# imjaegyun/Traffic-Context-Augmented-Vehicle-Trajectory-Prediction-Framework-Using-Multimodal-LLM

Hardware: AMD Instinct MI355X
Metric: trajectories/sec (higher is better)
Workload: dtype f16

## Files before the change

### include/tcavt.h

```cpp
#ifndef TCAVT_H
#define TCAVT_H

#include <stdint.h>

#ifdef __cplusplus
extern "C" {
#endif

typedef void* tcavt_stream_t;

#define TCAVT_ABI_VERSION 5

#define TCAVT_OK 0
#define TCAVT_ERR_ARG 1
#define TCAVT_ERR_HIP 2
#define TCAVT_ERR_ARCH 3

#define TCAVT_F32 0
#define TCAVT_BF16 1
#define TCAVT_F16 2

int tcavt_abi_version(void);
const char* tcavt_last_error(void);
int tcavt_init(int device, int* num_cus);
// ... 58 lines not shown

int tcavt_gemm_bf16(const tcavt_gemm_args* args, tcavt_stream_t stream);

int tcavt_rmsnorm(const float* x, const float* gamma, float eps, void* out_bf16,
                  float* out_f32, int M, int H, void* out_drop_bf16, float dropout_p,
                  uint64_t dropout_seed, uint32_t dropout_site, int dtype16 ,
                  tcavt_stream_t stream);

int tcavt_layernorm(const float* x, const float* residual, const float* gamma,
                    const float* beta, float eps, float* out_f32, void* out_bf16,
                    int M, int D, int dtype16 , tcavt_stream_t stream);

int tcavt_dropout(const void* x, void* out, int64_t n, int dtype, float p, uint64_t seed, uint32_t site,
                  const void* add ,
                  tcavt_stream_t stream);

int tcavt_set_dropout_epoch(const uint64_t* epoch_dev);
int tcavt_dropout_epoch_advance(uint64_t* epoch_dev, tcavt_stream_t stream);

int tcavt_copy_batch(void* const* dst, const void* const* src, const int64_t* bytes, int n, tcavt_stream_t stream);

int tcavt_cast_f32_16(const float* x, void* out16, int64_t n, int dtype16, tcavt_stream_t stream);

int tcavt_embed_fuse(const void* table_bf16, const int64_t* ids, const float* img,
                     const float* vis_mod, const float* txt_mod, float* h, int B,
                     int Nq, int Lt, int H, int V, int* bad_id_flag, int table_dtype,
                     void* h16, float* part, int npart, float stream_scale ,
                     tcavt_stream_t stream);

int tcavt_mask_to_kvlen(const int64_t* mask, int B, int Lt, int Nq, int32_t* kv_len,
                        int* not_prefix_flag, tcavt_stream_t stream);

int tcavt_attn_causal_gqa(const void* qkv, void* out, const int32_t* kv_len, int B,
                          int L, int nq, int nkv, float scale, int dtype16, tcavt_stream_t stream);
int tcavt_attn_causal_gqa_lse(const void* qkv, void* out, float* lse, const int32_t* kv_len, int B,
                              int L, int nq, int nkv, float scale, int dtype16, tcavt_stream_t stream);

int tcavt_softmax_rows(const float* S, int64_t lds, void* P, int64_t ldp, int out_dtype, int rows,
                       int n_valid, int n_out, float dropout_p, uint64_t dropout_seed, uint32_t dropout_site,
                       tcavt_stream_t stream);

int tcavt_mha(const void* q, int64_t ldq, const void* k, int64_t ldk, const void* v,
              int64_t ldv, void* out, int64_t ldo, const int32_t* key_len, int B,
              int Lq, int Lk, int nh, int dh, float scale, int in_dtype,
              int out_dtype, float dropout_p, uint64_t dropout_seed, uint32_t dropout_site,
              tcavt_stream_t stream);

int tcavt_gemm_f32(const float* A, int64_t lda, const float* W, int64_t ldw,
                   const float* bias, const float* residual, int64_t ldr, float* C,
                   int64_t ldc, int M, int N, int K, int flags, float dropout_p,
                   uint64_t dropout_seed, uint32_t dropout_site, tcavt_stream_t stream);

int tcavt_poly_embed(const float* polygon, const float* w_in, const float* b_in,
                     const float* pos, float* x, int B, int P, int D,
                     tcavt_stream_t stream);
int tcavt_masked_mean(const float* enc, const int32_t* len, float* emb, int B, int P,
                      int D, tcavt_stream_t stream);

int tcavt_ltsf_front(const float* x, const float* conv_w, const float* conv_b,
                     const float* enc_w, const float* enc_b, const float* pos,
                     float* enc_tok, float* xp_tok ,
                     int B, int C, int T, tcavt_stream_t stream);

int tcavt_ltsf_decode(const float* e_tok, const float* dec_w, const float* dec_b,
                      const float* lane_adj, float* dec, int B, int C, int T, int To,
                      tcavt_stream_t stream);

int tcavt_transpose_ct(const float* in, float* out_f32, void* out_bf16, int B, int C,
                       int To, int dtype16, tcavt_stream_t stream);

int tcavt_out_head(const float* fused, const float* w, const float* bias,
                   const float* x, float* out, int B, int To, int C, int F, int T,
                   int add_last, tcavt_stream_t stream);

int tcavt_traj_metrics(const float* pred, const float* gt, const float* norm_stat,
                       float* sums, int32_t* argmin, float* per_sample, int B, int K,
                       int To, tcavt_stream_t stream);

int tcavt_gemm_f32_strided(const float* A, int64_t rsA, int64_t csA, const float* W, int64_t rsW,
                           int64_t csW, const float* bias, const float* residual, int64_t ldr, float* C,
                           int64_t ldc, int M, int N, int K, int flags, float* ws, int64_t ws_elems,
                           tcavt_stream_t stream);


int tcavt_transpose16(const void* in, int64_t ld_in, void* out, int64_t ld_out, int rows, int cols,
                      int rows_pad, int batch, int64_t s_in, int64_t s_out, int f16_to_bf16, tcavt_stream_t stream);
int tcavt_transpose_f32_bf16(const float* in, int64_t ld_in, void* out, int64_t ld_out, int rows,
                             int cols, int rows_pad, tcavt_stream_t stream);
int tcavt_colsum(const void* g, int64_t ld, int dtype, float* out, int M, int N, int accumulate,
                 float* ws, int64_t ws_elems, tcavt_stream_t stream);
int tcavt_relu_bwd(float* g, const void* y, int y_dtype, int64_t n, tcavt_stream_t stream);
int tcavt_add_inplace(float* a, const float* b, int64_t n, tcavt_stream_t stream);
int tcavt_silu_mul_bwd(const void* gu_bf16, const void* g_act_bf16, void* g_gu_bf16, int64_t M, int I, int dtype16,
                       tcavt_stream_t stream);
int tcavt_rmsnorm_bwd(const void* x, const float* gamma, const void* gy_bf16, const void* gy2_bf16, float eps,
                      float* gx, void* gx_bf16, int accumulate, int M, int H, int gy_dtype, int out_dtype,
                      const float* gy_scale, int x_dtype, tcavt_stream_t stream);
int tcavt_grad_scale_pick(const void* g_a, const void* g_b, int64_t n, int dtype16, float target, float* scale,
                          uint32_t* scratch, const int32_t* backoff, tcavt_stream_t stream);
int tcavt_rope_bwd_pack(const float* g32, void* out_bf16, const float* rope_cos, const float* rope_sin, int64_t M,
                        int ncols, int rope_cols, int L, int dtype16, tcavt_stream_t stream);
int tcavt_attn_causal_gqa_bwd(const void* qkv_bf16, const void* dO_bf16, float* g32, const int32_t* kv_len, int B, int T,
                              int nq, int nkv, int head_dim, float scale, tcavt_stream_t stream);
int tcavt_causal_softmax_bwd_rows(const float* S, const float* dP, void* P_bf16, void* dS_bf16, const int32_t* kv_len,
                                  int B, int T, int Tp, int nq, float scale, tcavt_stream_t stream);
int tcavt_causal_softmax_bwd_tiles(const float* S, const float* dP, void* dS_bf16, void* PT_bf16, void* dST_bf16,
                                   const int32_t* kv_len, int B, int T, int Tp, int nq, float scale, tcavt_stream_t stream);
int tcavt_attn_bwd_scores(const void* qkv_bf16, const void* dO_bf16, void* dS_bf16, void* PT_bf16, void* dST_bf16,
                          float* dQ, int64_t ld_dq, float* stats, const int32_t* kv_len, int B, int T, int Tp, int nq,
                          int nkv, int head_dim, float scale, int dtype16, const float* lse, const void* att,
                          tcavt_stream_t stream);
int tcavt_attn_bwd_resident_ok(int T, int nq, int nkv);
int tcavt_attn_bwd_resident(const void* qkv16, const void* dO16, const void* att16, const float* lse, void* g_qkv16,
                            float* stats, const float* rope_cos, const float* rope_sin, const int32_t* kv_len, int B, int T,
                            int nq, int nkv, int head_dim, float scale, int dtype16, tcavt_stream_t stream);
int tcavt_attn_bwd_long_ok(int T, int nq, int nkv);
int tcavt_attn_bwd_long(const void* qkv16, const void* dO16, const void* att16, const float* lse, void* g_qkv16, float* stats,
                        const float* rope_cos, const float* rope_sin, const int32_t* kv_len, int B, int T, int nq, int nkv,
                        int head_dim, float scale, int dtype16, tcavt_stream_t stream);
int tcavt_attn_bwd_dkv(const void* qkv_bf16, const void* dO_bf16, const float* stats, float* g32, const int32_t* kv_len,
                       int B, int T, int Tp, int nq, int nkv, int head_dim, float scale, int dtype16, tcavt_stream_t stream);
int tcavt_gqa_rope_bwd_pack(const float* G3, void* out_bf16, const float* rope_cos, const float* rope_sin, int64_t M,
                            int nq, int nkv, int head_dim, int L, tcavt_stream_t stream);
int tcavt_wgrad_tn(const void* G, int64_t ldg, int g_col0, int n, const void* X, int64_t ldx, int x_dtype, float* C,
                   int64_t ldc, int M, int H, int trans_out, int g_dtype, const float* rs_part, int rs_npart, int rs_h,
                   float rs_eps, tcavt_stream_t stream);
int tcavt_lora_wgrad_a(const void* x16, const float* part, int npart, float eps, const float* gamma, const void* g_t, float* dA,
                       int64_t ldc, int M, int H, float dropout_p, uint64_t dropout_seed, uint32_t site_q, uint32_t site_v,
                       int dtype16, tcavt_stream_t stream);

int tcavt_clip_grad_norm(float* g, int64_t n, float max_norm, float grad_scale, float* scratch, tcavt_stream_t stream);
int tcavt_layernorm_bwd(const float* x, const float* gamma, const float* gy, float eps, float* gx,
                        float* ggamma, float* gbeta, int M, int D, float* ws, int64_t ws_elems, tcavt_stream_t stream);
int tcavt_mha_bwd(const float* q, int64_t ldq, const float* k, int64_t ldk, const float* v, int64_t ldv,
                  const float* go, int64_t ldo, float* gq, float* gk, float* gv, int64_t ldg,
                  const int32_t* key_len, int B, int Lq, int Lk, int nh, int dh, float scale,
                  float dropout_p, uint64_t dropout_seed, uint32_t dropout_site,
                  tcavt_stream_t stream);
int tcavt_softmax_bwd_rows(const void* P_f16, int64_t ldp, const float* dP, int64_t ldd, void* dS_bf16,
                           int64_t lds, float scale, int rows, int n_valid, int n_out,
                           tcavt_stream_t stream);
int tcavt_mse_grad(const float* pred, const float* gt, const float* norm_stat, float* g, int B, int To,
                   tcavt_stream_t stream);
int tcavt_mse_grad_seeded(const float* pred, const float* gt, const float* norm_stat, const float* g_loss,
                          const float* g_pred, float* g, int B, int To, tcavt_stream_t stream);
int tcavt_out_head_bwd(const float* g, const float* fused, const float* w, float* gf, float* gw, float* gb,
                       int B, int To, int C, int F, tcavt_stream_t stream);
int tcavt_nlinear_bwd(const float* in_tok, const float* W, const float* g, int64_t g_sb, int64_t g_sc,
                      int64_t g_ss, float* gW, float* gbias, float* gin_tok, int B, int C, int T, int S,
                      tcavt_stream_t stream);
int tcavt_conv1x1_bwd(const float* gxp_tok, const float* x, float* gw, float* gb, int B, int C, int T,
                      int F, tcavt_stream_t stream);
int tcavt_poly_embed_bwd(const float* g, const float* polygon, float* gw, float* gb, float* gpos, int B,
                         int P, int D, tcavt_stream_t stream);
int tcavt_masked_mean_bwd(const float* gemb, const int32_t* len, float* genc, int B, int P, int D,
                          tcavt_stream_t stream);
int tcavt_adamw(float* p, const float* g, float* m, float* v, int64_t n, float lr, float beta1, float beta2,
                float eps, float weight_decay, int step, float grad_scale, tcavt_stream_t stream);

typedef struct tcavt_llama_layer {
  const void* w_qkv;
  const void* a_cat;
  const void* b_ext;
  const void* w_o;
  const void* w_gu;
  const void* w_d;
  float* tape_h_mid;
  float* tape_h_out;
  void* tape_qkv;
  void* tape_gu;
  void* tape_t;
  void* tape_att;
  float* tape_lse;
  float* tape_part;
} tcavt_llama_layer;

typedef struct tcavt_llama_stack_args {
  const tcavt_llama_layer* layers;
  const float* gamma_final;
  const float* rope_cos;
  const float* rope_sin;
  float* h;
  void* h16;
  float* part;
  const int32_t* kv_len;
  void* qkv;
  void* att;
  void* act;
  void* t;
  void* xq;
  void* xv;
  float* out_f32;
  void* out16;
  void* k_cache;
  void* v_cache;
  void* const* events;
  int32_t n_layers, B, L, H, I, nq, nkv, dtype16;
  int32_t kv_lmax;
  int32_t gemm_tile;
  int32_t npart_in;
  float stream_scale;
  float rms_eps, lora_scale;
  float lora_dropout_p;
  uint32_t lora_first_site;
  uint64_t dropout_seed;
  int32_t* nonfinite_flag;
  void* splitk_ws;
  int64_t splitk_ws_bytes;
} tcavt_llama_stack_args;
// ... 377 lines not shown
```

### traffic-context-augmented-vehicle-trajectory-prediction-framework-using-multimodal-llm_amd/capi.py

```python
import ctypes
import os

import torch

_HERE = os.path.dirname(os.path.abspath(__file__))
LIB_PATH = os.path.join(_HERE, "libtcavt_hip.so")

ABI_VERSION = 5
F32, BF16, F16 = 0, 1, 2
EPI_BIAS, EPI_RELU, EPI_RESIDUAL, EPI_SILU_MUL, EPI_ROPE, EPI_BIAS_ROW, EPI_ACCUM = 1, 2, 4, 8, 16, 32, 64
EPI_NORM_OUT, EPI_ROWSCALE, EPI_SILU_BWD = 128, 256, 512
ACT_A_FRAG16, ACT_OUT_FRAG16, ACT_BLOCK8 = 1, 2, 4
W_FRAG16 = 1

c_void_p, c_int, c_int64, c_float = ctypes.c_void_p, ctypes.c_int, ctypes.c_int64, ctypes.c_float


class GemmArgs(ctypes.Structure):

    _fields_ = [
        ("A", c_void_p), ("lda", c_int64),
        ("W", c_void_p), ("ldw", c_int64),
        ("A2", c_void_p), ("lda2", c_int64),
        ("W2", c_void_p), ("ldw2", c_int64),
        ("C", c_void_p), ("ldc", c_int64),
        ("bias", c_void_p),
        ("residual", c_void_p), ("ldr", c_int64),
        ("rope_cos", c_void_p),
        ("rope_sin", c_void_p),
        ("M", ctypes.c_int32), ("N", ctypes.c_int32), ("K", ctypes.c_int32), ("K2", ctypes.c_int32),
        ("out_dtype", ctypes.c_int32),
        ("epilogue", ctypes.c_int32),
        ("rope_L", ctypes.c_int32), ("rope_cols", ctypes.c_int32),
        ("tile", ctypes.c_int32),
        ("acc_scale", ctypes.c_float),
        ("in_dtype", ctypes.c_int32),
        ("batch", ctypes.c_int32), ("batch_inner", ctypes.c_int32),
        ("sAo", c_int64), ("sAi", c_int64), ("sWo", c_int64), ("sWi", c_int64), ("sCo", c_int64), ("sCi", c_int64),
        ("dropout_p", ctypes.c_float), ("dropout_site", ctypes.c_uint32), ("dropout_seed", ctypes.c_uint64),
        ("batch_w_group", ctypes.c_int32), ("w_layout", ctypes.c_int32),
        ("silu_preact", c_void_p), ("ld_preact", c_int64),
        ("norm_h16", c_void_p), ("norm_part", c_void_p), ("rowscale_part", c_void_p),
        ("rowscale_npart", ctypes.c_int32), ("rowscale_h", ctypes.c_int32), ("rowscale_eps", ctypes.c_float),
        ("norm_scale", ctypes.c_float),
        ("rope_pos", c_void_p),
        ("nonfinite_flag", c_void_p), ("nonfinite_tag", ctypes.c_int32), ("act_layout", ctypes.c_int32),
        ("norm_res16", c_void_p), ("splitk_ws", c_void_p), ("splitk_ws_bytes", c_int64),
        ("lora_part", c_void_p), ("lora_part_a", c_void_p), ("lora_part_lda", c_int64), ("lora_part_np", c_int),
        ("lora_part_scale", c_float),
    ]


class LlamaLayer(ctypes.Structure):

    _fields_ = [(n, c_void_p) for n in ("w_qkv", "a_cat", "b_ext", "w_o", "w_gu", "w_d", "tape_h_mid", "tape_h_out",
                                        "tape_qkv", "tape_gu", "tape_t", "tape_att", "tape_lse", "tape_part")]


TLAYER_FIELDS = ("w_in", "b_in", "w_out", "b_out", "w_q", "b_q", "w_kv", "b_kv", "w_co", "b_co", "w1", "b1", "w2", "b2",
                 "n1_w", "n1_b", "n2_w", "n2_b", "n3_w", "n3_b",
                 "qkv", "att", "y", "x1", "x1b", "cq", "ckv", "catt", "cy", "x2", "x2b", "ffh", "y2", "out", "outb")


class TLayer(ctypes.Structure):

    _fields_ = [(n, c_void_p) for n in TLAYER_FIELDS]


class TStackArgs(ctypes.Structure):

    _fields_ = [
        ("layers", ctypes.POINTER(TLayer)),
        ("x", c_void_p), ("xb", c_void_p), ("mem", c_void_p), ("memb", c_void_p), ("key_len", c_void_p),
        ("n_layers", ctypes.c_int32), ("B", ctypes.c_int32), ("L", ctypes.c_int32), ("Lk", ctypes.c_int32),
        ("E", ctypes.c_int32), ("FF", ctypes.c_int32), ("nhead", ctypes.c_int32), ("dtype16", ctypes.c_int32),
        ("dropout_p", ctypes.c_float), ("first_site", ctypes.c_uint32), ("dropout_seed", ctypes.c_uint64),
    ]


class CrossAttnArgs(ctypes.Structure):

    _fields_ = [(n, c_void_p) for n in ("q", "wk_t", "w_v", "b_v", "fh", "fh_t", "qp", "scores", "probs", "ctx", "att")] + [
        (n, ctypes.c_int32) for n in ("B", "To", "L", "Lp", "H", "nhead", "dtype16")] + [
        ("dropout_p", ctypes.c_float), ("dropout_site", ctypes.c_uint32), ("reserved0", ctypes.c_uint32),
        ("dropout_seed", ctypes.c_uint64)]


class TLayerGrads(ctypes.Structure):

    _fields_ = [(n, c_void_p) for n in ("g_w_in", "g_b_in", "g_w_out", "g_b_out", "g_w1", "g_b1", "g_w2", "g_b2", "g_n1_w", "g_n1_b",
                                        "g_n2_w", "g_n2_b")]


class TStackBwdArgs(ctypes.Structure):

    _fields_ = [("fwd", ctypes.POINTER(TStackArgs)), ("grads", ctypes.POINTER(TLayerGrads))] + [(n, c_void_p) for n in (
        "g_out", "g_x", "g_tmp", "g_y2", "g_y2d", "g_x1", "g_y", "g_yd", "g_att", "g_f", "g_qkv")] + [
        ("red_ws", c_void_p), ("red_ws_elems", c_int64)]
# ... 62 lines not shown
        ("g_h", c_void_p), ("g_hb", c_void_p), ("g_xn", c_void_p), ("g_xl", c_void_p), ("g_att", c_void_p),
        ("g_qkv0", c_void_p), ("g_qkv1", c_void_p), ("g_t0", c_void_p), ("g_t1", c_void_p),
        ("dA", c_void_p), ("dB", c_void_p), ("stats", c_void_p),
        ("leaf_stream", c_void_p), ("events", ctypes.POINTER(c_void_p)),
        ("n_layers", ctypes.c_int32), ("B", ctypes.c_int32), ("L", ctypes.c_int32), ("H", ctypes.c_int32),
        ("I", ctypes.c_int32), ("nq", ctypes.c_int32), ("nkv", ctypes.c_int32), ("dtype16", ctypes.c_int32),
        ("npart", ctypes.c_int32), ("lora_rank", ctypes.c_int32), ("input_grad", ctypes.c_int32), ("reserved0", ctypes.c_int32),
        ("rms_eps", ctypes.c_float), ("lora_scale", ctypes.c_float), ("lora_dropout_p", ctypes.c_float),
        ("lora_first_site", ctypes.c_uint32), ("dropout_seed", ctypes.c_uint64), ("scale_backoff", c_void_p),
    ]


class SampleParams(ctypes.Structure):

    _fields_ = [("temperature", c_float), ("top_p", c_float), ("repetition_penalty", c_float), ("top_k", ctypes.c_int32),
                ("no_repeat_ngram_size", ctypes.c_int32), ("do_sample", ctypes.c_int32), ("eos_token_id", c_int64),
                ("pad_token_id", c_int64), ("seed", ctypes.c_uint64)]


class DecodeArgs(ctypes.Structure):

    _fields_ = [("layers", ctypes.POINTER(LlamaLayer))] + [(n, c_void_p) for n in (
        "gamma_final", "rope_cos", "rope_sin", "table", "txt_mod", "cur_tok", "pos", "h", "h16", "part", "qkv", "att", "act",
        "t", "k_cache", "v_cache", "x16", "logits", "bad_id_flag")] + [(n, ctypes.c_int32) for n in (
            "n_layers", "B", "H", "I", "nq", "nkv", "V", "dtype16", "kv_lmax", "rope_L")] + [
        ("rms_eps", c_float), ("lora_scale", c_float), ("nonfinite_flag", c_void_p), ("splitk_ws", c_void_p),
        ("splitk_ws_bytes", c_int64), ("lora_part", c_void_p), ("lora_rank", c_int), ("stream_scale", ctypes.c_float),
        ("w_layout", ctypes.c_int32), ("act_layout", ctypes.c_int32), ("table_packed", c_void_p)]


class LmLossArgs(ctypes.Structure):

    _fields_ = [("h16", c_void_p), ("ldh", c_int64), ("table", c_void_p), ("table_t", c_void_p), ("ldt", c_int64),
                ("labels", c_void_p), ("kv_len", c_void_p)] + [(n, ctypes.c_int32) for n in (
                    "B", "L", "V", "H", "Nq", "dtype16", "grad_dtype", "reserved0")] + [(n, c_void_p) for n in (
                        "loss", "count", "lse", "row_loss", "flag", "g_loss", "g_out")] + [
        ("ldg", c_int64), ("workspace", c_void_p), ("workspace_bytes", c_int64)]


class LmEvalArgs(ctypes.Structure):

    _fields_ = [("h16", c_void_p), ("ldh", c_int64), ("table", c_void_p), ("labels", c_void_p), ("kv_len", c_void_p)] + [
        (n, ctypes.c_int32) for n in ("B", "L", "V", "H", "Nq", "dtype16")] + [(n, c_void_p) for n in (
            "loss", "count", "lse", "row_loss", "flag", "pred", "correct", "sample_tokens", "sample_correct", "sample_nll")] + [
        ("workspace", c_void_p), ("workspace_bytes", c_int64)]


_SIGNATURES = {
    "tcavt_abi_version": [],
    "tcavt_last_error": [],
    "tcavt_init": [c_int, ctypes.POINTER(c_int)],
    "tcavt_gemm_bf16": [ctypes.POINTER(GemmArgs), c_void_p],
    "tcavt_rmsnorm": [c_void_p, c_void_p, c_float, c_void_p, c_void_p, c_int, c_int, c_void_p, c_float, ctypes.c_uint64,
                      ctypes.c_uint32, c_int, c_void_p],
    "tcavt_layernorm": [c_void_p, c_void_p, c_void_p, c_void_p, c_float, c_void_p, c_void_p, c_int, c_int, c_int, c_void_p],
    "tcavt_cast_f32_16": [c_void_p, c_void_p, c_int64, c_int, c_void_p],
    "tcavt_copy_batch": [c_void_p, c_void_p, c_void_p, c_int, c_void_p],
    "tcavt_embed_fuse": [c_void_p, c_void_p, c_void_p, c_void_p, c_void_p, c_void_p, c_int, c_int, c_int, c_int,
                         c_int, c_void_p, c_int, c_void_p, c_void_p, c_int, c_float, c_void_p],
    "tcavt_softmax_rows": [c_void_p, c_int64, c_void_p, c_int64, c_int, c_int, c_int, c_int, c_float, ctypes.c_uint64,
                           ctypes.c_uint32, c_void_p],
    "tcavt_set_dropout_epoch": [c_void_p],
    "tcavt_dropout_epoch_advance": [c_void_p, c_void_p],
    "tcavt_dropout": [c_void_p, c_void_p, c_int64, c_int, c_float, ctypes.c_uint64, ctypes.c_uint32, c_void_p, c_void_p],
    "tcavt_mask_to_kvlen": [c_void_p, c_int, c_int, c_int, c_void_p, c_void_p, c_void_p],
    "tcavt_attn_causal_gqa": [c_void_p, c_void_p, c_void_p, c_int, c_int, c_int, c_int, c_float, c_int, c_void_p],
    "tcavt_attn_causal_gqa_lse": [c_void_p, c_void_p, c_void_p, c_void_p, c_int, c_int, c_int, c_int, c_float, c_int, c_void_p],
    "tcavt_mha": [c_void_p, c_int64, c_void_p, c_int64, c_void_p, c_int64, c_void_p, c_int64, c_void_p, c_int,
                  c_int, c_int, c_int, c_int, c_float, c_int, c_int, c_float, ctypes.c_uint64, ctypes.c_uint32, c_void_p],
    "tcavt_gemm_f32": [c_void_p, c_int64, c_void_p, c_int64, c_void_p, c_void_p, c_int64, c_void_p, c_int64,
                       c_int, c_int, c_int, c_int, c_float, ctypes.c_uint64, ctypes.c_uint32, c_void_p],
    "tcavt_poly_embed": [c_void_p, c_void_p, c_void_p, c_void_p, c_void_p, c_int, c_int, c_int, c_void_p],
    "tcavt_masked_mean": [c_void_p, c_void_p, c_void_p, c_int, c_int, c_int, c_void_p],
    "tcavt_ltsf_front": [c_void_p, c_void_p, c_void_p, c_void_p, c_void_p, c_void_p, c_void_p, c_void_p, c_int, c_int,
                         c_int, c_void_p],
    "tcavt_ltsf_decode": [c_void_p, c_void_p, c_void_p, c_void_p, c_void_p, c_int, c_int, c_int, c_int, c_void_p],
    "tcavt_transpose_ct": [c_void_p, c_void_p, c_void_p, c_int, c_int, c_int, c_int, c_void_p],
    "tcavt_out_head": [c_void_p, c_void_p, c_void_p, c_void_p, c_void_p, c_int, c_int, c_int, c_int, c_int,
                       c_int, c_void_p],
    "tcavt_traj_metrics": [c_void_p, c_void_p, c_void_p, c_void_p, c_void_p, c_void_p, c_int, c_int, c_int,
                           c_void_p],
    "tcavt_gemm_f32_strided": [c_void_p, c_int64, c_int64, c_void_p, c_int64, c_int64, c_void_p, c_void_p, c_int64,
                               c_void_p, c_int64, c_int, c_int, c_int, c_int, c_void_p, c_int64, c_void_p],
    "tcavt_transpose16": [c_void_p, c_int64, c_void_p, c_int64, c_int, c_int, c_int, c_int, c_int64, c_int64, c_int, c_void_p],
    "tcavt_transpose_f32_bf16": [c_void_p, c_int64, c_void_p, c_int64, c_int, c_int, c_int, c_void_p],
    "tcavt_colsum": [c_void_p, c_int64, c_int, c_void_p, c_int, c_int, c_int, c_void_p, c_int64, c_void_p],
    "tcavt_relu_bwd": [c_void_p, c_void_p, c_int, c_int64, c_void_p],
    "tcavt_add_inplace": [c_void_p, c_void_p, c_int64, c_void_p],
    "tcavt_silu_mul_bwd": [c_void_p, c_void_p, c_void_p, c_int64, c_int, c_int, c_void_p],
    "tcavt_rmsnorm_bwd": [c_void_p, c_void_p, c_void_p, c_void_p, c_float, c_void_p, c_void_p, c_int, c_int, c_int, c_int, c_int,
                          c_void_p, c_int, c_void_p],
    "tcavt_lora_dgrad": [c_void_p, c_void_p, c_void_p, c_void_p, c_int, c_int, c_float, ctypes.c_uint64, ctypes.c_uint32,
                         ctypes.c_uint32, c_int, c_void_p],
    "tcavt_grad_scale_pick": [c_void_p, c_void_p, c_int64, c_int, c_float, c_void_p, c_void_p, c_void_p, c_void_p],
    "tcavt_rope_bwd_pack": [c_void_p, c_void_p, c_void_p, c_void_p, c_int64, c_int, c_int, c_int, c_int, c_void_p],
    "tcavt_attn_causal_gqa_bwd": [c_void_p, c_void_p, c_void_p, c_void_p, c_int, c_int, c_int, c_int, c_int, c_float,
                                  c_void_p],
    "tcavt_causal_softmax_bwd_rows": [c_void_p, c_void_p, c_void_p, c_void_p, c_void_p, c_int, c_int, c_int, c_int, c_float,
                                      c_void_p],
    "tcavt_causal_softmax_bwd_tiles": [c_void_p, c_void_p, c_void_p, c_void_p, c_void_p, c_void_p, c_int, c_int, c_int, c_int,
                                       c_float, c_void_p],
    "tcavt_attn_bwd_scores": [c_void_p, c_void_p, c_void_p, c_void_p, c_void_p, c_void_p, c_int64, c_void_p, c_void_p, c_int,
                              c_int, c_int, c_int, c_int, c_int, c_float, c_int, c_void_p, c_void_p, c_void_p],
    "tcavt_attn_bwd_resident_ok": [c_int, c_int, c_int],
    "tcavt_attn_bwd_resident": [c_void_p, c_void_p, c_void_p, c_void_p, c_void_p, c_void_p, c_void_p, c_void_p, c_void_p, c_int,
                                c_int, c_int, c_int, c_int, c_float, c_int, c_void_p],
    "tcavt_attn_bwd_long_ok": [c_int, c_int, c_int],
    "tcavt_attn_bwd_long": [c_void_p, c_void_p, c_void_p, c_void_p, c_void_p, c_void_p, c_void_p, c_void_p, c_void_p, c_int,
                            c_int, c_int, c_int, c_int, c_float, c_int, c_void_p],
    "tcavt_attn_bwd_dkv": [c_void_p, c_void_p, c_void_p, c_void_p, c_void_p, c_int, c_int, c_int, c_int, c_int, c_int, c_float,
                           c_int, c_void_p],
    "tcavt_gqa_rope_bwd_pack": [c_void_p, c_void_p, c_void_p, c_void_p, c_int64, c_int, c_int, c_int, c_int, c_void_p],
    "tcavt_wgrad_tn": [c_void_p, c_int64, c_int, c_int, c_void_p, c_int64, c_int, c_void_p, c_int64, c_int, c_int, c_int, c_int,
                       c_void_p, c_int, c_int, c_float, c_void_p],
    "tcavt_lora_wgrad_a": [c_void_p, c_void_p, c_int, c_float, c_void_p, c_void_p, c_void_p, c_int64, c_int, c_int, c_float,
                           ctypes.c_uint64, ctypes.c_uint32, ctypes.c_uint32, c_int, c_void_p],
    "tcavt_clip_grad_norm": [c_void_p, c_int64, c_float, c_float, c_void_p, c_void_p],
    "tcavt_layernorm_bwd": [c_void_p, c_void_p, c_void_p, c_float, c_void_p, c_void_p, c_void_p, c_int, c_int, c_void_p,
                            c_int64, c_void_p],
    "tcavt_mha_bwd": [c_void_p, c_int64, c_void_p, c_int64, c_void_p, c_int64, c_void_p, c_int64, c_void_p, c_void_p,
                      c_void_p, c_int64, c_void_p, c_int, c_int, c_int, c_int, c_int, c_float, c_float, ctypes.c_uint64,
                      ctypes.c_uint32, c_void_p],
    "tcavt_softmax_bwd_rows": [c_void_p, c_int64, c_void_p, c_int64, c_void_p, c_int64, c_float, c_int, c_int, c_int,
                               c_void_p],
    "tcavt_mse_grad": [c_void_p, c_void_p, c_void_p, c_void_p, c_int, c_int, c_void_p],
    "tcavt_mse_grad_seeded": [c_void_p, c_void_p, c_void_p, c_void_p, c_void_p, c_void_p, c_int, c_int, c_void_p],
    "tcavt_out_head_bwd": [c_void_p, c_void_p, c_void_p, c_void_p, c_void_p, c_void_p, c_int, c_int, c_int, c_int,
                           c_void_p],
    "tcavt_nlinear_bwd": [c_void_p, c_void_p, c_void_p, c_int64, c_int64, c_int64, c_void_p, c_void_p, c_void_p, c_int,
                          c_int, c_int, c_int, c_void_p],
    "tcavt_conv1x1_bwd": [c_void_p, c_void_p, c_void_p, c_void_p, c_int, c_int, c_int, c_int, c_void_p],
    "tcavt_poly_embed_bwd": [c_void_p, c_void_p, c_void_p, c_void_p, c_void_p, c_int, c_int, c_int, c_void_p],
    "tcavt_masked_mean_bwd": [c_void_p, c_void_p, c_void_p, c_int, c_int, c_int, c_void_p],
    "tcavt_adamw": [c_void_p, c_void_p, c_void_p, c_void_p, c_int64, c_float, c_float, c_float, c_float, c_float,
                    c_int, c_float, c_void_p],
    "tcavt_llama_stack_forward": [ctypes.POINTER(LlamaStackArgs), c_void_p],
    "tcavt_sample_logits": [c_void_p, c_int, c_int, c_void_p, c_int, c_void_p, ctypes.POINTER(SampleParams), c_void_p, c_void_p,
                            c_void_p, c_void_p, c_void_p, c_int, c_int, c_void_p, c_int64, c_void_p],
    "tcavt_sample_workspace_bytes": [c_int],
    "tcavt_gather_last": [c_void_p, c_void_p, c_void_p, c_int, c_int, c_int, c_void_p],
    "tcavt_llama_decode_step": [ctypes.POINTER(DecodeArgs), c_void_p],
    "tcavt_norm_npart": [c_int, c_int, c_int],
    "tcavt_pack_weight16": [c_void_p, c_int64, c_void_p, c_int, c_int, c_void_p],
    "tcavt_lora_down": [c_void_p, c_void_p, c_void_p, c_int, c_int, c_float, c_float, ctypes.c_uint64, ctypes.c_uint32,
                        ctypes.c_uint32, c_int, c_void_p],
    "tcavt_rownorm_prep": [c_void_p, c_void_p, c_void_p, c_int64, c_int, c_int, c_int, c_int, c_float, c_void_p],
    "tcavt_allreduce_flat": [c_void_p, c_int64, c_void_p, c_void_p],
    "tcavt_tlayer_stack_forward": [ctypes.POINTER(TStackArgs), c_void_p],
    "tcavt_cross_attn_forward": [ctypes.POINTER(CrossAttnArgs), c_void_p],
    "tcavt_ltsf_forward": [ctypes.POINTER(LtsfArgs), c_int, c_void_p],
    "tcavt_cross_attn_backward": [ctypes.POINTER(CrossAttnBwdArgs), c_void_p],
    "tcavt_ltsf_backward": [ctypes.POINTER(LtsfBwdArgs), c_int, c_void_p],
    "tcavt_tlayer_stack_backward": [ctypes.POINTER(TStackBwdArgs), c_void_p],
    "tcavt_rmsnorm16": [c_void_p, c_void_p, c_float, c_void_p, c_void_p, c_int, c_int, c_int, c_void_p],
    "tcavt_llama_stack_backward": [ctypes.POINTER(LlamaBackwardArgs), c_void_p],
    "tcavt_events_create": [ctypes.POINTER(c_void_p), c_int],
    "tcavt_events_destroy": [ctypes.POINTER(c_void_p), c_int],
    "tcavt_event_elapsed_ms": [c_void_p, c_void_p, ctypes.POINTER(c_float)],
    "tcavt_adamw_gated": [c_void_p, c_void_p, c_void_p, c_void_p, c_int64, c_float, c_float, c_float, c_float, c_float,
                          c_float, c_void_p, c_void_p, c_void_p, c_void_p],
    "tcavt_lm_loss_workspace_bytes": [c_int64, c_int, c_int],
    "tcavt_lm_loss_forward": [ctypes.POINTER(LmLossArgs), c_void_p],
    "tcavt_lm_loss_backward": [ctypes.POINTER(LmLossArgs), c_void_p],
    "tcavt_lm_eval_workspace_bytes": [c_int64, c_int, c_int],
    "tcavt_lm_eval": [ctypes.POINTER(LmEvalArgs), c_void_p],
}
_RESTYPES = {"tcavt_last_error": ctypes.c_char_p, "tcavt_sample_workspace_bytes": c_int64,
             "tcavt_lm_loss_workspace_bytes": c_int64, "tcavt_lm_eval_workspace_bytes": c_int64}

EXPORTED_SYMBOLS = tuple(_SIGNATURES)


class TcavtError(RuntimeError):
    pass


_lib = None


def lib():
    global _lib
    if _lib is not None:
        return _lib
    if not os.path.exists(LIB_PATH):
        raise TcavtError(
            f"{LIB_PATH} not found: the HIP extension is not built. Run "
            "`python -c 'import __graft_entry__ as g; g.build()'` (or `python -m tcavt_amd.build`). "
            "There is no CPU/PyTorch fallback for the hot path."
        )
    handle = ctypes.CDLL(LIB_PATH)
    for name, argtypes in _SIGNATURES.items():
        fn = getattr(handle, name)
        fn.argtypes = argtypes
        fn.restype = _RESTYPES.get(name, c_int)
    if handle.tcavt_abi_version() != ABI_VERSION:
        raise TcavtError("libtcavt_hip.so ABI version mismatch")
    _lib = handle
# ... 28 lines not shown
```

### traffic-context-augmented-vehicle-trajectory-prediction-framework-using-multimodal-llm_amd/csrc/llm_backward.hip

```cpp
#include "common.hpp"
#include "philox.hpp"
#include <stdlib.h>

namespace tcavt {

__device__ __forceinline__ float sigmoid_f(float g) { return __builtin_amdgcn_rcpf(1.f + __expf(-g)); }

template <bool F16>
__device__ __forceinline__ f32x4 mfma16b(const bf16x8& a, const bf16x8& b, const f32x4& c) {
  if constexpr (F16) return __builtin_amdgcn_mfma_f32_16x16x32_f16(__builtin_bit_cast(f16x8, a), __builtin_bit_cast(f16x8, b), c, 0, 0, 0);
  else return __builtin_amdgcn_mfma_f32_16x16x32_bf16(a, b, c, 0, 0, 0);
}
template <bool F16>
__device__ __forceinline__ float half16(unsigned int w, int k) { return k ? from16_hi<F16>(w) : from16_lo<F16>(w); }

template <bool F16>
__global__ __launch_bounds__(256) void silu_mul_bwd_kernel(const bf16_t* __restrict__ gu, const bf16_t* __restrict__ g_act,
                                                           bf16_t* __restrict__ g_gu, long M, int I) {
  const long blk = (long)blockIdx.x * blockDim.x + threadIdx.x;
  const long nblk = M * (I >> 4);
  if (blk >= nblk) return;
  const u32x4* src = reinterpret_cast<const u32x4*>(gu + blk * 32);
  const u32x4* dsrc = reinterpret_cast<const u32x4*>(g_act + blk * 16);
  u32x4 gv[2] = {src[0], src[1]}, uv[2] = {src[2], src[3]}, dv[2] = {dsrc[0], dsrc[1]};
// ... 1424 lines not shown
    for (int b = 0; b < 4; ++b) acc[a][b] = f32x4{0.f, 0.f, 0.f, 0.f};
  const int tp = tid >> 4, cc = (tid & 15) * 16;
  const int grow = tid >> 2, gc0 = (tid & 3) * 8;
  for (int m0 = mbeg; m0 < mend; m0 += 32) {
    {
      u32x4 v[2][2];
#pragma unroll
      for (int r = 0; r < 2; ++r) {
        const int m = m0 + 2 * tp + r;
#pragma unroll
        for (int o = 0; o < 2; ++o) {
          v[r][o] = u32x4{0u, 0u, 0u, 0u};
          if (m < mend && h0 + cc + 8 * o < H) v[r][o] = *reinterpret_cast<const u32x4*>(X + (long)m * H + h0 + cc + 8 * o);
        }
      }
      u32x4 gv = {0u, 0u, 0u, 0u};
      if (tid < 128 && m0 + grow < mend) gv = *reinterpret_cast<const u32x4*>(Gt + (long)(m0 + grow) * 64 + gc0);
      if (tid < 32) rs_s[tid] = m0 + tid < mend ? part_rscale(part + (long)(m0 + tid) * npart, npart, inv_h, eps) : 0.f;
      __syncthreads();
      const float rs2[2] = {rs_s[2 * tp], rs_s[2 * tp + 1]};
#pragma unroll
      for (int o = 0; o < 2; ++o) {
        u32x4 wq[2], wv[2];
#pragma unroll
        for (int r = 0; r < 2; ++r) {
          float sq[8], sv[8];
          if (drop) {
            const unsigned long long oct =
                ((unsigned long long)(m0 + 2 * tp + r) * (unsigned long long)H + (unsigned long long)(h0 + cc + 8 * o)) >> 3;
            dropout_oct(dq, oct, sq);
            dropout_oct(dv, oct, sv);
          }
#pragma unroll
          for (int e = 0; e < 4; ++e) {
            const float lo = from16_lo<F16>(v[r][o][e]) * rs2[r], hi = from16_hi<F16>(v[r][o][e]) * rs2[r];
            wq[r][e] = drop ? pack16x2<F16>(lo * sq[2 * e], hi * sq[2 * e + 1]) : pack16x2<F16>(lo, hi);
            if (drop) wv[r][e] = pack16x2<F16>(lo * sv[2 * e], hi * sv[2 * e + 1]);
          }
        }
#pragma unroll
        for (int e = 0; e < 4; ++e) {
          const int c = cc + 8 * o + 2 * e;
          *reinterpret_cast<unsigned int*>(&xq[c * XS + 2 * tp]) = (wq[0][e] & 0xffffu) | (wq[1][e] << 16);
          *reinterpret_cast<unsigned int*>(&xq[(c + 1) * XS + 2 * tp]) = (wq[0][e] >> 16) | (wq[1][e] & 0xffff0000u);
          if (drop) {
            *reinterpret_cast<unsigned int*>(&xv[c * XS + 2 * tp]) = (wv[0][e] & 0xffffu) | (wv[1][e] << 16);
            *reinterpret_cast<unsigned int*>(&xv[(c + 1) * XS + 2 * tp]) = (wv[0][e] >> 16) | (wv[1][e] & 0xffff0000u);
          }
        }
      }
      if (tid < 128) {
#pragma unroll
        for (int e = 0; e < 4; ++e) {
          gt[(gc0 + 2 * e) * XS + grow] = static_cast<bf16_t>(gv[e] & 0xffffu);
          gt[(gc0 + 2 * e + 1) * XS + grow] = static_cast<bf16_t>(gv[e] >> 16);
        }
      }
    }
    __syncthreads();
    const u32x4 aq = *reinterpret_cast<const u32x4*>(&gt[r16 * XS + kq * 8]);
    const u32x4 av = *reinterpret_cast<const u32x4*>(&gt[(16 + r16) * XS + kq * 8]);
#pragma unroll
    for (int b = 0; b < 4; ++b) {
      const int row = (wave * 64 + b * 16 + r16) * XS + kq * 8;
      const u32x4 bq = *reinterpret_cast<const u32x4*>(&xq[row]);
      const u32x4 bv = *reinterpret_cast<const u32x4*>(&xvp[row]);
      acc[0][b] = mfma16b<F16>(__builtin_bit_cast(bf16x8, aq), __builtin_bit_cast(bf16x8, bq), acc[0][b]);
      acc[1][b] = mfma16b<F16>(__builtin_bit_cast(bf16x8, av), __builtin_bit_cast(bf16x8, bv), acc[1][b]);
    }
    __syncthreads();
  }
#pragma unroll
  for (int a = 0; a < 2; ++a)
#pragma unroll
    for (int b = 0; b < 4; ++b) {
      const int h = h0 + wave * 64 + b * 16 + r16;
      if (h >= H) continue;
      const float gm = gamma[h];
#pragma unroll
      for (int e = 0; e < 4; ++e) atomicAdd(dA + (long)(a * 16 + 4 * kq + e) * ldc + h, acc[a][b][e] * gm);
    }
}

template <bool XF16, bool GF16 = false>
__global__ __launch_bounds__(256) void wgrad_tn_kernel(const bf16_t* __restrict__ G, long ldg, int g0, int NB,
                                                       const bf16_t* __restrict__ X, long ldx, float* __restrict__ C,
                                                       long ldc, int M, int H, int m_per_wg, int trans_out,
                                                       const float* __restrict__ rs_part, int rs_npart, float rs_inv_h,
                                                       float rs_eps) {
  constexpr int XS = 40;
  __shared__ __attribute__((aligned(16))) bf16_t xt[256 * XS];
  __shared__ __attribute__((aligned(16))) bf16_t gt[64 * XS];
  const int tid = threadIdx.x, lane = tid & 63, wave = tid >> 6;
  const int h0 = blockIdx.x * 256;
  const int mbeg = blockIdx.y * m_per_wg, mend = min(mbeg + m_per_wg, M);
  const int r16 = lane & 15, kq = lane >> 4;
  f32x4 acc[4][4];
#pragma unroll
  for (int a = 0; a < 4; ++a)
#pragma unroll
    for (int b = 0; b < 4; ++b) acc[a][b] = f32x4{0.f, 0.f, 0.f, 0.f};
  const int xrow = tid >> 3, xc0 = (tid & 7) * 32;
  const int grow = tid >> 3, gc0 = (tid & 7) * 8;
  for (int m0 = mbeg; m0 < mend; m0 += 32) {
    {
      const int m = m0 + xrow;
      const bool ok = m < mend;
#pragma unroll
      for (int c = 0; c < 4; ++c) {
        u32x4 v = {0u, 0u, 0u, 0u};
        const int col = h0 + xc0 + c * 8;
        if (ok && col < H) v = *reinterpret_cast<const u32x4*>(X + (long)m * ldx + col);
#pragma unroll
        for (int e = 0; e < 4; ++e) {
          bf16_t lo = static_cast<bf16_t>(v[e] & 0xffffu), hi = static_cast<bf16_t>(v[e] >> 16);
          if constexpr (XF16 && !GF16) {
            lo = f32_to_bf16(f16_to_f32(lo));
            hi = f32_to_bf16(f16_to_f32(hi));
          }
          xt[(xc0 + c * 8 + 2 * e) * XS + xrow] = lo;
          xt[(xc0 + c * 8 + 2 * e + 1) * XS + xrow] = hi;
        }
      }
      if (gc0 < 16 * NB) {
        u32x4 v = {0u, 0u, 0u, 0u};
        const int mg = m0 + grow;
        if (mg < mend) v = *reinterpret_cast<const u32x4*>(G + (long)mg * ldg + g0 + gc0);
        if (rs_part && mg < mend) {
          const float rs = part_rscale(rs_part + (long)mg * rs_npart, rs_npart, rs_inv_h, rs_eps);
#pragma unroll
          for (int e = 0; e < 4; ++e) v[e] = pack16x2<GF16>(from16_lo<GF16>(v[e]) * rs, from16_hi<GF16>(v[e]) * rs);
        }
#pragma unroll
        for (int e = 0; e < 4; ++e) {
          gt[(gc0 + 2 * e) * XS + grow] = static_cast<bf16_t>(v[e] & 0xffffu);
          gt[(gc0 + 2 * e + 1) * XS + grow] = static_cast<bf16_t>(v[e] >> 16);
        }
      }
    }
    __syncthreads();
    u32x4 bf[4];
#pragma unroll
    for (int b = 0; b < 4; ++b) bf[b] = *reinterpret_cast<const u32x4*>(&xt[(wave * 64 + b * 16 + r16) * XS + kq * 8]);
#pragma unroll
    for (int a = 0; a < 4; ++a) {
      if (a < NB) {
        const u32x4 af = *reinterpret_cast<const u32x4*>(&gt[(a * 16 + r16) * XS + kq * 8]);
#pragma unroll
        for (int b = 0; b < 4; ++b)
          acc[a][b] = mfma16b<GF16>(__builtin_bit_cast(bf16x8, af), __builtin_bit_cast(bf16x8, bf[b]), acc[a][b]);
      }
    }
    __syncthreads();
  }
#pragma unroll
  for (int a = 0; a < 4; ++a) {
    if (a >= NB) continue;
#pragma unroll
    for (int b = 0; b < 4; ++b) {
      const int h = h0 + wave * 64 + b * 16 + r16;
      if (h >= H) continue;
#pragma unroll
      for (int e = 0; e < 4; ++e) {
        const int n = a * 16 + 4 * kq + e;
        float* dst = trans_out ? C + (long)h * ldc + n : C + (long)n * ldc + h;
        atomicAdd(dst, acc[a][b][e]);
      }
    }
  }
}

__global__ __launch_bounds__(256) void adapter_grads_out_kernel(float* __restrict__ dA, float* __restrict__ dB, float* __restrict__ gAq,
                                                                float* __restrict__ gAv, float* __restrict__ gBq, float* __restrict__ gBv,
                                                                int H, int nqkv, int q_rows, int v_row0, int r,
                                                                const float* __restrict__ scale) {
  const long idx = (long)blockIdx.x * blockDim.x + threadIdx.x;
  const long nA = (long)64 * H;
  const float sc = scale ? *scale : 1.f;
  if (idx < nA) {
    const int i = (int)(idx / H), j = (int)(idx - (long)i * H);
    const float v = dA[idx];
    dA[idx] = 0.f;
    if (i < r) gAq[(long)i * H + j] = v * sc;
    else if (i >= 16 && i < 16 + r) gAv[(long)(i - 16) * H + j] = v * sc;
    return;
  }
  const long k = idx - nA;
  if (k >= (long)nqkv * 64) return;
  const int i = (int)(k >> 6), j = (int)(k & 63);
  const float v = dB[k];
  dB[k] = 0.f;
  if (i < q_rows && j < r) gBq[(long)i * r + j] = v * sc;
  else if (i >= v_row0 && j >= 16 && j < 16 + r) gBv[(long)(i - v_row0) * r + (j - 16)] = v * sc;
}

template <bool F16>
__global__ __launch_bounds__(256) void grad_amax_kernel(const bf16_t* __restrict__ a, const bf16_t* __restrict__ b, long n8,
                                                        unsigned int* __restrict__ amax_bits) {
  float m = 0.f;
  for (long i = (long)blockIdx.x * blockDim.x + threadIdx.x; i < n8; i += (long)gridDim.x * blockDim.x) {
    const u32x4 v = reinterpret_cast<const u32x4*>(a)[i];
#pragma unroll
    for (int e = 0; e < 4; ++e) m = fmaxf(m, fmaxf(fabsf(from16_lo<F16>(v[e])), fabsf(from16_hi<F16>(v[e]))));
    if (b) {
      const u32x4 w = reinterpret_cast<const u32x4*>(b)[i];
#pragma unroll
      for (int e = 0; e < 4; ++e) m = fmaxf(m, fmaxf(fabsf(from16_lo<F16>(w[e])), fabsf(from16_hi<F16>(w[e]))));
    }
  }
  m = wave_max(m);
  if ((threadIdx.x & 63) == 0 && m > 0.f) atomicMax(amax_bits, __float_as_uint(m));
}
__global__ void grad_scale_set_kernel(unsigned int* __restrict__ amax_bits, float target, float* __restrict__ scale,
                                      const int* __restrict__ backoff) {
  const float m = __uint_as_float(*amax_bits);
  float s = 1.f;
  if (m > 0.f && m < 3.0e38f) {
    int e;
    (void)frexpf(target / m, &e);
    e = max(-60, min(60, e - 1 - (backoff ? *backoff : 0)));
    s = ldexpf(1.f, e);
  }
  scale[0] = s;
  scale[1] = 1.f / s;
  *amax_bits = 0u;
}

}

using namespace tcavt;

extern "C" int tcavt_silu_mul_bwd(const void* gu_bf16, const void* g_act_bf16, void* g_gu_bf16, int64_t M, int I, int dtype16,
                                  tcavt_stream_t stream) {
  TCAVT_CHECK_ARG(is16(dtype16), "silu_mul_bwd: dtype16 must be TCAVT_BF16 or TCAVT_F16");
  TCAVT_CHECK_ARG(gu_bf16 && g_act_bf16 && g_gu_bf16 && M > 0 && I > 0 && I % 16 == 0, "silu_mul_bwd: bad args (I %% 16 == 0)");
  TCAVT_CHECK_ARG(aligned16(gu_bf16) && aligned16(g_act_bf16) && aligned16(g_gu_bf16), "silu_mul_bwd: 16-byte alignment required");
  const long n = (long)M * (I / 16);
  auto kfn = dtype16 == TCAVT_F16 ? silu_mul_bwd_kernel<true> : silu_mul_bwd_kernel<false>;
  hipLaunchKernelGGL(kfn, dim3((unsigned)((n + 255) / 256)), dim3(256), 0, static_cast<hipStream_t>(stream),
                     static_cast<const bf16_t*>(gu_bf16), static_cast<const bf16_t*>(g_act_bf16),
                     static_cast<bf16_t*>(g_gu_bf16), (long)M, I);
  TCAVT_CHECK_LAUNCH("silu_mul_bwd");
  return TCAVT_OK;
}

extern "C" int tcavt_rmsnorm_bwd(const void* x, const float* gamma, const void* gy_bf16, const void* gy2_bf16, float eps,
                                 float* gx, void* gx_bf16, int accumulate, int M, int H, int gy_dtype, int out_dtype,
                                 const float* gy_scale, int x_dtype, tcavt_stream_t stream) {
  TCAVT_CHECK_ARG(is16(gy_dtype) && (gx_bf16 == nullptr || is16(out_dtype)), "rmsnorm_bwd: gy_dtype / out_dtype must be TCAVT_BF16 or TCAVT_F16");
  TCAVT_CHECK_ARG(x_dtype == TCAVT_F32 || is16(x_dtype), "rmsnorm_bwd: x_dtype must be TCAVT_F32, TCAVT_F16 or TCAVT_BF16");
// ... 344 lines not shown
                                   a->dropout_seed, site, site + 1, dt, lf));
      TCAVT_TRY(tcavt_wgrad_tn(w.t, 64, 0, 32, g_qkv2[par], nqkv, dt, a->dB, 64, M, nqkv, 1, dt, w.part, a->npart, H, a->rms_eps, lf));
      const long n_out = (long)64 * H + (long)nqkv * 64;
      hipLaunchKernelGGL(adapter_grads_out_kernel, dim3((unsigned)((n_out + 255) / 256)), dim3(256), 0, lf, a->dA, a->dB, w.g_Aq, w.g_Av,
                         w.g_Bq, w.g_Bv, H, nqkv, nq * 64, (nq + nkv) * 64, r, f16 ? inv_s : nullptr);
      TCAVT_CHECK_LAUNCH("llama_stack_backward(adapter gradients)");
    }
    if (two) {
      TCAVT_TRY(hip_ok(hipEventRecord(static_cast<hipEvent_t>(a->events[2 + par]), lf), "record(done)"));
      leaf_used[par] = true;
    }
    if (li == 0 && !a->input_grad) break;
    {
      const uint32_t site = a->lora_first_site + 2u * (uint32_t)li;
      TCAVT_TRY(tcavt_lora_dgrad(g_t2[par], w.a_qT, w.a_vT, a->g_xl, M, H, a->lora_dropout_p, a->dropout_seed, site, site + 1, dt, stream));
    }
    TCAVT_TRY(gemm(g_qkv2[par], nqkv, w.w_qkvT, nqkv, a->g_xn, H, 0.f));
    TCAVT_TRY(tcavt_rmsnorm_bwd(w.h_in, w.g1, a->g_xn, a->g_xl, a->rms_eps, a->g_h, a->g_hb, 1, M, H, dt, dt, nullptr, dt, stream));
  }
  return TCAVT_OK;
  };
  const int rc_walk = walk();
  int rc_join = TCAVT_OK;
  if (two) {
    if (rc_walk != TCAVT_OK) {
      if (hipEventRecord(static_cast<hipEvent_t>(a->events[2]), lf) == hipSuccess) leaf_used[0] = true;
    }
    for (int par = 0; par < 2; ++par)
      if (leaf_used[par] && hipStreamWaitEvent(st, static_cast<hipEvent_t>(a->events[2 + par]), 0) != hipSuccess && rc_walk == TCAVT_OK) {
        set_error("llama_stack_backward: join(leaf) failed");
        rc_join = TCAVT_ERR_HIP;
      }
  }
  return rc_walk != TCAVT_OK ? rc_walk : rc_join;
}

extern "C" int tcavt_clip_grad_norm(float* g, int64_t n, float max_norm, float grad_scale, float* scratch,
                                    tcavt_stream_t stream) {
  TCAVT_CHECK_ARG(g && scratch && n > 0 && max_norm > 0.f && grad_scale > 0.f, "clip_grad_norm: bad args");
  hipStream_t st = static_cast<hipStream_t>(stream);
  hipLaunchKernelGGL(sumsq_partial_kernel, dim3(CLIP_BLOCKS), dim3(256), 0, st, g, (long)n, scratch);
  hipLaunchKernelGGL(clip_scale_kernel, dim3(1), dim3(64), 0, st, scratch, max_norm, grad_scale);
  long blocks = (n + 255) / 256;
  if (blocks > 4096) blocks = 4096;
  hipLaunchKernelGGL(scale_by_kernel, dim3((unsigned)blocks), dim3(256), 0, st, g, (long)n, scratch + CLIP_BLOCKS);
  TCAVT_CHECK_LAUNCH("clip_grad_norm");
  return TCAVT_OK;
}

extern "C" int tcavt_wgrad_tn(const void* G, int64_t ldg, int g_col0, int n, const void* X, int64_t ldx, int x_dtype, float* C,
                              int64_t ldc, int M, int H, int trans_out, int g_dtype, const float* rs_part, int rs_npart, int rs_h,
                              float rs_eps, tcavt_stream_t stream) {
  TCAVT_CHECK_ARG(!rs_part || (rs_npart > 0 && rs_npart % 4 == 0 && rs_h > 0 && aligned16(rs_part)),
                  "wgrad_tn: rs_part needs rs_npart %% 4 == 0, rs_h > 0 and 16-byte alignment");
  const float rs_inv_h = rs_part ? 1.f / (float)rs_h : 0.f;
  TCAVT_CHECK_ARG(G && X && C && M > 0 && H > 0 && n > 0 && n <= 64 && n % 16 == 0 && g_col0 >= 0 && g_col0 % 8 == 0 &&
                      ldg % 8 == 0 && ldx % 8 == 0 && H % 8 == 0 && is16(x_dtype),
                  "wgrad_tn: n in {16, 32, 48, 64}, g_col0 / ldg / ldx / H multiples of 8");
  TCAVT_CHECK_ARG(g_dtype == 0 || g_dtype == TCAVT_BF16 || (g_dtype == TCAVT_F16 && x_dtype == TCAVT_F16),
                  "wgrad_tn: G is bf16 (g_dtype 0 / TCAVT_BF16), or fp16 together with an fp16 X");
  TCAVT_CHECK_ARG(aligned16(G) && aligned16(X), "wgrad_tn: 16-byte alignment required");
  const int gx = (H + 255) / 256;
  int split = 256 / gx;
  if (split < 1) split = 1;
  int m_per_wg = ((M + split - 1) / split + 31) / 32 * 32;
  split = (M + m_per_wg - 1) / m_per_wg;
  const dim3 grid(gx, split), block(256);
  if (g_dtype == TCAVT_F16)
    hipLaunchKernelGGL((wgrad_tn_kernel<true, true>), grid, block, 0, static_cast<hipStream_t>(stream), static_cast<const bf16_t*>(G),
                       (long)ldg, g_col0, n / 16, static_cast<const bf16_t*>(X), (long)ldx, C, (long)ldc, M, H, m_per_wg, trans_out,
                       rs_part, rs_npart, rs_inv_h, rs_eps);
  else if (x_dtype == TCAVT_F16)
    hipLaunchKernelGGL(wgrad_tn_kernel<true>, grid, block, 0, static_cast<hipStream_t>(stream), static_cast<const bf16_t*>(G),
                       (long)ldg, g_col0, n / 16, static_cast<const bf16_t*>(X), (long)ldx, C, (long)ldc, M, H, m_per_wg, trans_out,
                       rs_part, rs_npart, rs_inv_h, rs_eps);
  else
    hipLaunchKernelGGL(wgrad_tn_kernel<false>, grid, block, 0, static_cast<hipStream_t>(stream), static_cast<const bf16_t*>(G),
                       (long)ldg, g_col0, n / 16, static_cast<const bf16_t*>(X), (long)ldx, C, (long)ldc, M, H, m_per_wg, trans_out,
                       rs_part, rs_npart, rs_inv_h, rs_eps);
  TCAVT_CHECK_LAUNCH("wgrad_tn");
  return TCAVT_OK;
}

extern "C" int tcavt_lora_wgrad_a(const void* x16, const float* part, int npart, float eps, const float* gamma, const void* g_t,
                                  float* dA, int64_t ldc, int M, int H, float dropout_p, uint64_t dropout_seed, uint32_t site_q,
                                  uint32_t site_v, int dtype16, tcavt_stream_t stream) {
  TCAVT_CHECK_ARG(x16 && part && gamma && g_t && dA && M > 0 && H > 0 && H % 16 == 0 && npart > 0 && npart % 4 == 0 && ldc >= H &&
                      is16(dtype16) && dropout_p >= 0.f && dropout_p < 1.f,
                  "lora_wgrad_a: bad args (H %% 16 == 0, npart %% 4 == 0, ldc >= H, 0 <= dropout_p < 1)");
  TCAVT_CHECK_ARG(aligned16(x16) && aligned16(part) && aligned16(g_t), "lora_wgrad_a: 16-byte alignment required");
  const DropoutP dq = make_dropout(dropout_p, dropout_seed, site_q), dv = make_dropout(dropout_p, dropout_seed, site_v);
  const int gx = (H + 255) / 256;
  int split = 256 / gx;
  if (split < 1) split = 1;
  int m_per_wg = ((M + split - 1) / split + 31) / 32 * 32;
  split = (M + m_per_wg - 1) / m_per_wg;
  auto kfn = dtype16 == TCAVT_F16 ? lora_wgrad_a_kernel<true> : lora_wgrad_a_kernel<false>;
  hipLaunchKernelGGL(kfn, dim3(gx, split), dim3(256), 0, static_cast<hipStream_t>(stream), static_cast<const bf16_t*>(x16), part, npart,
                     1.f / (float)H, eps, gamma, static_cast<const bf16_t*>(g_t), dA, (long)ldc, M, H, m_per_wg, dq, dv);
  TCAVT_CHECK_LAUNCH("lora_wgrad_a");
  return TCAVT_OK;
}

extern "C" int tcavt_grad_scale_pick(const void* g_a, const void* g_b, int64_t n, int dtype16, float target, float* scale,
                                     uint32_t* scratch, const int32_t* backoff, tcavt_stream_t stream) {
  TCAVT_CHECK_ARG(g_a && scale && scratch && n > 0 && n % 8 == 0 && is16(dtype16) && target > 0.f && aligned16(g_a) && aligned16(g_b),
                  "grad_scale_pick: bad args (n %% 8 == 0, 16-byte alignment, scratch = one zero-initialised uint32)");
  hipStream_t st = static_cast<hipStream_t>(stream);
  long blocks = (n / 8 + 255) / 256;
  if (blocks > 1024) blocks = 1024;
  auto kfn = dtype16 == TCAVT_F16 ? grad_amax_kernel<true> : grad_amax_kernel<false>;
  hipLaunchKernelGGL(kfn, dim3((unsigned)blocks), dim3(256), 0, st, static_cast<const bf16_t*>(g_a), static_cast<const bf16_t*>(g_b),
                     (long)(n / 8), scratch);
  hipLaunchKernelGGL(grad_scale_set_kernel, dim3(1), dim3(1), 0, st, scratch, target, scale, backoff);
  TCAVT_CHECK_LAUNCH("grad_scale_pick");
  return TCAVT_OK;
}
```

### traffic-context-augmented-vehicle-trajectory-prediction-framework-using-multimodal-llm_amd/csrc/small.hip

```cpp
#include "common.hpp"
#include "philox.hpp"

namespace tcavt {

__device__ __forceinline__ void gemm_f32_fetch(const float* __restrict__ X, long rs, long cs, int r0, int R, int k0,
                                               int K, int tid, bool kfast, float (&v)[4], int (&row)[4], int (&kk)[4]) {
#pragma unroll
  for (int e = 0; e < 4; ++e) {
    const int idx = e * 256 + tid;
    const int r = kfast ? (idx >> 4) : (idx & 63);
    const int k = kfast ? (idx & 15) : (idx >> 6);
    row[e] = r;
    kk[e] = k;
    const int gr = r0 + r, gk = k0 + k;
    v[e] = (gr < R && gk < K) ? X[(long)gr * rs + (long)gk * cs] : 0.f;
  }
}

__global__ __launch_bounds__(256) void gemm_f32_kernel(const float* __restrict__ A, long rsA, long csA,
                                                       const float* __restrict__ W, long rsW, long csW,
                                                       const float* __restrict__ bias,
                                                       const float* __restrict__ res, long ldr,
                                                       float* __restrict__ C, long ldc, int M, int N,
                                                       int K, int flags, int k_chunk, DropoutP drop,
                                                       float* __restrict__ part) {
  const int kb = blockIdx.z * k_chunk, ke = min(K, kb + k_chunk);
  __shared__ float As[64][17];
  __shared__ float Ws[64][17];
  const int tid = threadIdx.x, lane = tid & 63, wave = tid >> 6;
  const int wm = wave >> 1, wn = wave & 1;
  const int m0 = blockIdx.y * 64, n0 = blockIdx.x * 64;
  const bool akf = csA <= rsA, wkf = csW <= rsW;
  f32x4 acc[2][2];
#pragma unroll
  for (int i = 0; i < 2; ++i)
#pragma unroll
    for (int j = 0; j < 2; ++j) acc[i][j] = f32x4{0.f, 0.f, 0.f, 0.f};
  float va[4], vw[4];
  int ra[4], ka[4], rw[4], kw[4];
  gemm_f32_fetch(A, rsA, csA, m0, M, kb, ke, tid, akf, va, ra, ka);
  gemm_f32_fetch(W, rsW, csW, n0, N, kb, ke, tid, wkf, vw, rw, kw);
  const int lr = lane & 15, lk = lane >> 4;
  for (int k0 = kb; k0 < ke; k0 += 16) {
#pragma unroll
    for (int e = 0; e < 4; ++e) {
      As[ra[e]][ka[e]] = va[e];
      Ws[rw[e]][kw[e]] = vw[e];
    }
    __syncthreads();
    if (k0 + 16 < ke) {
      gemm_f32_fetch(A, rsA, csA, m0, M, k0 + 16, ke, tid, akf, va, ra, ka);
      gemm_f32_fetch(W, rsW, csW, n0, N, k0 + 16, ke, tid, wkf, vw, rw, kw);
    }
#pragma unroll
    for (int ks = 0; ks < 4; ++ks) {
      float af[2], wf[2];
#pragma unroll
      for (int i = 0; i < 2; ++i) af[i] = As[wm * 32 + i * 16 + lr][ks * 4 + lk];
#pragma unroll
      for (int j = 0; j < 2; ++j) wf[j] = Ws[wn * 32 + j * 16 + lr][ks * 4 + lk];
#pragma unroll
      for (int i = 0; i < 2; ++i)
#pragma unroll
        for (int j = 0; j < 2; ++j) acc[i][j] = __builtin_amdgcn_mfma_f32_16x16x4f32(af[i], wf[j], acc[i][j], 0, 0, 0);
    }
    __syncthreads();
  }
#pragma unroll
  for (int i = 0; i < 2; ++i)
#pragma unroll
    for (int j = 0; j < 2; ++j) {
      const int n = n0 + wn * 32 + j * 16 + lr;
      if (n >= N) continue;
#pragma unroll
      for (int r = 0; r < 4; ++r) {
        const int m = m0 + wm * 32 + i * 16 + 4 * lk + r;
        if (m >= M) continue;
        float v = acc[i][j][r];
        if (gridDim.z > 1) {
          if (part) {
            part[((long)blockIdx.z * M + m) * N + n] = v;
            continue;
          }
          if (blockIdx.z == 0) {
            if (flags & TCAVT_EPI_BIAS) v += bias[n];
            if (flags & TCAVT_EPI_RESIDUAL) v += res[(long)m * ldr + n];
          }
          atomicAdd(&C[(long)m * ldc + n], v);
          continue;
        }
        if (flags & TCAVT_EPI_ACCUM) v += C[(long)m * ldc + n];
        if (flags & TCAVT_EPI_BIAS) v += bias[n];
        if (flags & TCAVT_EPI_RELU) v = relu_nan(v);
        if (drop.p > 0.f) v *= dropout_one(drop, (unsigned long long)m * (unsigned long long)N + (unsigned long long)n);
        if (flags & TCAVT_EPI_RESIDUAL) v += res[(long)m * ldr + n];
        C[(long)m * ldc + n] = v;
      }
    }
}

__global__ void poly_embed_kernel(const float* __restrict__ poly, const float* __restrict__ w,
                                  const float* __restrict__ bi, const float* __restrict__ pos,
                                  float* __restrict__ x, int B, int P, int D) {
  const long idx = (long)blockIdx.x * blockDim.x + threadIdx.x;
  if (idx >= (long)B * P * D) return;
  const int d = (int)(idx % D);
  const long bp = idx / D;
  const int p = (int)(bp % P);
  const float px = poly[bp * 2], py = poly[bp * 2 + 1];
  x[idx] = fmaf(w[d * 2 + 1], py, fmaf(w[d * 2], px, 0.f)) + bi[d] + pos[p * D + d];
}

__global__ void masked_mean_kernel(const float* __restrict__ enc, const int* __restrict__ len,
                                   float* __restrict__ emb, int B, int P, int D) {
  const int idx = blockIdx.x * blockDim.x + threadIdx.x;
  if (idx >= B * D) return;
  const int b = idx / D, d = idx % D;
  const int n = min(len[b], P);
  float s = 0.f;
  for (int p = 0; p < n; ++p) s += enc[((long)b * P + p) * D + d];
  emb[idx] = n > 0 ? s / (float)n : 0.f;
}

__global__ void ltsf_front_kernel(const float* __restrict__ x, const float* __restrict__ cw,
                                  const float* __restrict__ cb, const float* __restrict__ ew,
                                  const float* __restrict__ eb, const float* __restrict__ pos,
                                  float* __restrict__ tok, float* __restrict__ xp_tok, int B, int C, int T) {
  extern __shared__ float xs[];
  const int b = blockIdx.x;
  for (int i = threadIdx.x; i < 2 * T; i += blockDim.x) xs[i] = x[(long)b * 2 * T + i];
  __syncthreads();
  for (int cs = threadIdx.x; cs < C * T; cs += blockDim.x) {
    const int c = cs / T, s = cs % T;
    const float w0 = cw[c * 2], w1 = cw[c * 2 + 1], bb = cb[c];
    const float last = fmaf(w1, xs[T + T - 1], fmaf(w0, xs[T - 1], 0.f)) + bb;
    float acc = 0.f;
    const float* wr = ew + ((long)c * T + s) * T;
    for (int t = 0; t < T; ++t) {
      const float xp = fmaf(w1, xs[T + t], fmaf(w0, xs[t], 0.f)) + bb;
      acc = fmaf(wr[t], xp - last, acc);
    }
    tok[((long)b * T + s) * C + c] = acc + eb[c * T + s] + last + pos[c * T + s];
    if (xp_tok) xp_tok[((long)b * T + s) * C + c] = fmaf(w1, xs[T + s], fmaf(w0, xs[s], 0.f)) + bb;
  }
}

__global__ void ltsf_decode_kernel(const float* __restrict__ e, const float* __restrict__ dw,
                                   const float* __restrict__ db, const float* __restrict__ lane,
                                   float* __restrict__ dec, int B, int C, int T, int To) {
// ... 28 lines not shown
  const int s = (int)(bs % To);
  const long b = bs / To;
  const float v = in[(b * C + c) * To + s];
  if (of) of[idx] = v;
  if (ob) ob[idx] = f16 ? f32_to_f16(v) : f32_to_bf16(v);
}

__global__ void out_head_kernel(const float* __restrict__ fused, const float* __restrict__ w,
                                const float* __restrict__ bias, const float* __restrict__ x,
                                float* __restrict__ out, int B, int To, int C, int F, int T, int add_last) {
  const int idx = blockIdx.x * blockDim.x + threadIdx.x;
  if (idx >= B * F * To) return;
  const int s = idx % To, f = (idx / To) % F, b = idx / (To * F);
  const float* fr = fused + ((long)b * To + s) * C;
  float acc = 0.f;
  for (int c = 0; c < C; ++c) acc = fmaf(w[f * C + c], fr[c], acc);
  out[idx] = acc + bias[f] + (add_last ? x[((long)b * F + f) * T + T - 1] : 0.f);
}

__global__ __launch_bounds__(1024) void traj_metrics_kernel(const float* __restrict__ pred,
                                                          const float* __restrict__ gt,
                                                          const float* __restrict__ ns,
                                                          float* __restrict__ sums,
                                                          int* __restrict__ argmin,
                                                          float* __restrict__ per_sample, int B, int K,
                                                          int To) {
  const int lane = threadIdx.x & 63, wave = threadIdx.x >> 6, nwave = blockDim.x >> 6;
  __shared__ float part[16][5];
  float acc0 = 0.f, acc1 = 0.f, acc2 = 0.f, acc3 = 0.f, acc4 = 0.f;
  for (int b = wave; b < B; b += nwave) {
  const float minx = ns[b * 4], maxx = ns[b * 4 + 1], miny = ns[b * 4 + 2], maxy = ns[b * 4 + 3];
  const float rx = maxx - minx, ry = maxy - miny;
  float best_ade = 0.f, best_fde = 0.f, best_rmse = 0.f;
  int ia = 0, ifd = 0, ir = 0;
  float sx_tot = 0.f, sy_tot = 0.f;
  for (int k = 0; k < K; ++k) {
    const float* px = pred + (((long)b * K + k) * 2) * To;
    const float* py = px + To;
    const float* gx = gt + (long)b * 2 * To;
    const float* gy = gx + To;
    float sx = 0.f, sy = 0.f, se = 0.f, last = 0.f;
    for (int t = lane; t < To; t += 64) {
      const float dx = (px[t] * rx + minx) - (gx[t] * rx + minx);
      const float dy = (py[t] * ry + miny) - (gy[t] * ry + miny);
      sx += dx * dx;
      sy += dy * dy;
      const float err = sqrtf(dx * dx + dy * dy);
      se += err;
      if (t == To - 1) last = err;
    }
    sx = wave_sum(sx);
    sy = wave_sum(sy);
    se = wave_sum(se);
    last = wave_sum(last);
    const float ade = se / (float)To;
    const float rmse = sqrtf((sx + sy) / (float)(2 * To));
    if (k == 0 || ade < best_ade) { best_ade = ade; ia = k; }
    if (k == 0 || last < best_fde) { best_fde = last; ifd = k; }
    if (k == 0 || rmse < best_rmse) { best_rmse = rmse; ir = k; }
    if (k == 0) { sx_tot = sx; sy_tot = sy; }
  }
  acc0 += sx_tot; acc1 += sy_tot; acc2 += best_ade; acc3 += best_fde; acc4 += best_rmse;
  if (lane == 0) {
    if (argmin) { argmin[b * 3] = ia; argmin[b * 3 + 1] = ifd; argmin[b * 3 + 2] = ir; }
    if (per_sample) { per_sample[b * 3] = best_ade; per_sample[b * 3 + 1] = best_fde; per_sample[b * 3 + 2] = best_rmse; }
  }
  }
  if (lane == 0) { part[wave][0] = acc0; part[wave][1] = acc1; part[wave][2] = acc2; part[wave][3] = acc3; part[wave][4] = acc4; }
  __syncthreads();
  if (threadIdx.x < 5) {
    float t = 0.f;
    for (int w = 0; w < nwave; ++w) t += part[w][threadIdx.x];
    sums[threadIdx.x] += t;
  }
}

}

using namespace tcavt;

__global__ __launch_bounds__(256) void splitk_reduce_f32_kernel(const float* __restrict__ part, int S,
                                                                const float* __restrict__ bias,
                                                                const float* __restrict__ res, long ldr, float* C,
                                                                long ldc, int M, int N, int flags) {
  const long i = (long)blockIdx.x * 256 + threadIdx.x;
  if (i >= (long)M * N) return;
  const int m = (int)(i / N), n = (int)(i % N);
  float v = part[i];
  for (int s = 1; s < S; ++s) v += part[(long)s * M * N + i];
  if (flags & TCAVT_EPI_ACCUM) v += C[(long)m * ldc + n];
  if (flags & TCAVT_EPI_BIAS) v += bias[n];
  if (flags & TCAVT_EPI_RESIDUAL) v += res[(long)m * ldr + n];
  C[(long)m * ldc + n] = v;
}

static int launch_gemm_f32(int max_splits, const float* A, long rsA, long csA, const float* W, long rsW, long csW, const float* bias,
                           const float* residual, long ldr, float* C, long ldc, int M, int N, int K, int flags,
                           DropoutP drop, float* ws, int64_t ws_elems, hipStream_t stream, const char* what) {
  const int tiles = ((N + 63) / 64) * ((M + 63) / 64);
  int splits = 1;
  if (tiles < 128 && K >= 512 && !(flags & TCAVT_EPI_RELU) && drop.p == 0.f) {
    int cap = 0;
    if (ws)
      cap = (int)std::min<int64_t>(max_splits, ws_elems / ((int64_t)M * N));
    else if (!(flags & TCAVT_EPI_ACCUM) && residual != C && ldc == N)
      cap = std::min(max_splits, 2);
    splits = std::min(K / 256, cap);
    while (splits > 1 && tiles * splits > 512) splits >>= 1;
    if (splits < 1) splits = 1;
  }
  int k_chunk = K;
  const bool partials = splits > 1 && ws;
  if (splits > 1) {
    k_chunk = (((K + splits - 1) / splits) + 15) / 16 * 16;
    splits = (K + k_chunk - 1) / k_chunk;
    if (!partials) {
      hipError_t e = hipMemsetAsync(C, 0, (size_t)M * N * sizeof(float), stream);
      if (e != hipSuccess) {
        set_error("%s: hipMemsetAsync failed: %s", what, hipGetErrorString(e));
        return TCAVT_ERR_HIP;
      }
    }
  }
  dim3 grid((N + 63) / 64, (M + 63) / 64, splits), block(256);
  hipLaunchKernelGGL(gemm_f32_kernel, grid, block, 0, stream, A, rsA, csA, W, rsW, csW, bias, residual, ldr, C, ldc, M,
                     N, K, flags, k_chunk, drop, splits > 1 && partials ? ws : nullptr);
  if (splits > 1 && partials)
    hipLaunchKernelGGL(splitk_reduce_f32_kernel, dim3((unsigned)(((int64_t)M * N + 255) / 256)), dim3(256), 0, stream, ws,
                       splits, bias, residual, ldr, C, ldc, M, N, flags);
  hipError_t e = hipGetLastError();
  if (e != hipSuccess) {
    set_error("%s: launch failed: %s", what, hipGetErrorString(e));
    return TCAVT_ERR_HIP;
  }
  return TCAVT_OK;
}

extern "C" int tcavt_gemm_f32(const float* A, int64_t lda, const float* W, int64_t ldw,
                              const float* bias, const float* residual, int64_t ldr, float* C,
                              int64_t ldc, int M, int N, int K, int flags, float dropout_p,
                              uint64_t dropout_seed, uint32_t dropout_site, tcavt_stream_t stream) {
  TCAVT_CHECK_ARG(A && W && C && M > 0 && N > 0 && K > 0, "gemm_f32: null pointer or bad shape");
  TCAVT_CHECK_ARG(dropout_p >= 0.f && dropout_p < 1.f, "gemm_f32: dropout_p must be in [0, 1)");
  TCAVT_CHECK_ARG(!(flags & TCAVT_EPI_BIAS) || bias, "gemm_f32: BIAS without bias");
  TCAVT_CHECK_ARG(!(flags & TCAVT_EPI_RESIDUAL) || residual, "gemm_f32: RESIDUAL without residual");
  TCAVT_CHECK_ARG(!(flags & ~(TCAVT_EPI_BIAS | TCAVT_EPI_RELU | TCAVT_EPI_RESIDUAL)), "gemm_f32: unsupported flag");
  return launch_gemm_f32(2, A, (long)lda, 1L, W, (long)ldw, 1L, bias, residual, (long)ldr, C, (long)ldc, M, N, K, flags,
                         make_dropout(dropout_p, dropout_seed, dropout_site), nullptr, 0, static_cast<hipStream_t>(stream),
                         "gemm_f32");
}

extern "C" int tcavt_gemm_f32_strided(const float* A, int64_t rsA, int64_t csA, const float* W, int64_t rsW,
                                      int64_t csW, const float* bias, const float* residual, int64_t ldr, float* C,
                                      int64_t ldc, int M, int N, int K, int flags, float* ws, int64_t ws_elems,
                                      tcavt_stream_t stream) {
  TCAVT_CHECK_ARG(A && W && C && M > 0 && N > 0 && K > 0, "gemm_f32_strided: null pointer or bad shape");
  TCAVT_CHECK_ARG(!(flags & TCAVT_EPI_BIAS) || bias, "gemm_f32_strided: BIAS without bias");
  TCAVT_CHECK_ARG(!(flags & TCAVT_EPI_RESIDUAL) || residual, "gemm_f32_strided: RESIDUAL without residual");
  TCAVT_CHECK_ARG(!(flags & ~(TCAVT_EPI_BIAS | TCAVT_EPI_RELU | TCAVT_EPI_RESIDUAL | TCAVT_EPI_ACCUM)), "gemm_f32_strided: unsupported flag");
  TCAVT_CHECK_ARG(!((flags & TCAVT_EPI_ACCUM) && (flags & TCAVT_EPI_RELU)), "gemm_f32_strided: ACCUM excludes RELU");
  return launch_gemm_f32(8, A, (long)rsA, (long)csA, W, (long)rsW, (long)csW, bias, residual, (long)ldr, C, (long)ldc, M,
                         N, K, flags, make_dropout(0.f, 0, 0), ws, ws_elems, static_cast<hipStream_t>(stream),
                         "gemm_f32_strided");
}

extern "C" int tcavt_poly_embed(const float* polygon, const float* w_in, const float* b_in,
                                const float* pos, float* x, int B, int P, int D, tcavt_stream_t stream) {
  TCAVT_CHECK_ARG(polygon && w_in && b_in && pos && x && B > 0 && P > 0 && D > 0, "poly_embed: bad args");
  const long n = (long)B * P * D;
  hipLaunchKernelGGL(poly_embed_kernel, dim3((unsigned)((n + 255) / 256)), dim3(256), 0,
                     static_cast<hipStream_t>(stream), polygon, w_in, b_in, pos, x, B, P, D);
  TCAVT_CHECK_LAUNCH("poly_embed");
  return TCAVT_OK;
}

extern "C" int tcavt_masked_mean(const float* enc, const int32_t* len, float* emb, int B, int P, int D,
                                 tcavt_stream_t stream) {
  TCAVT_CHECK_ARG(enc && len && emb && B > 0 && P > 0 && D > 0, "masked_mean: bad args");
  hipLaunchKernelGGL(masked_mean_kernel, dim3((B * D + 255) / 256), dim3(256), 0,
                     static_cast<hipStream_t>(stream), enc, len, emb, B, P, D);
  TCAVT_CHECK_LAUNCH("masked_mean");
  return TCAVT_OK;
}

extern "C" int tcavt_ltsf_front(const float* x, const float* conv_w, const float* conv_b,
                                const float* enc_w, const float* enc_b, const float* pos,
                                float* enc_tok, float* xp_tok, int B, int C, int T, tcavt_stream_t stream) {
  TCAVT_CHECK_ARG(x && conv_w && conv_b && enc_w && enc_b && pos && enc_tok && B > 0 && C > 0 && T > 0,
                  "ltsf_front: bad args");
  hipLaunchKernelGGL(ltsf_front_kernel, dim3(B), dim3(256), 2 * T * sizeof(float),
                     static_cast<hipStream_t>(stream), x, conv_w, conv_b, enc_w, enc_b, pos, enc_tok, xp_tok, B, C, T);
  TCAVT_CHECK_LAUNCH("ltsf_front");
  return TCAVT_OK;
}

extern "C" int tcavt_ltsf_decode(const float* e_tok, const float* dec_w, const float* dec_b,
                                 const float* lane_adj, float* dec, int B, int C, int T, int To,
                                 tcavt_stream_t stream) {
  TCAVT_CHECK_ARG(e_tok && dec_w && dec_b && lane_adj && dec && B > 0 && C > 0 && T > 0 && To > 0,
                  "ltsf_decode: bad args");
  TCAVT_CHECK_ARG((long)T * C * 4 <= 48 * 1024, "ltsf_decode: T*C too large for LDS");
  hipLaunchKernelGGL(ltsf_decode_kernel, dim3((C * To + 255) / 256, B), dim3(256), T * C * sizeof(float),
                     static_cast<hipStream_t>(stream), e_tok, dec_w, dec_b, lane_adj, dec, B, C, T, To);
  TCAVT_CHECK_LAUNCH("ltsf_decode");
  return TCAVT_OK;
}

extern "C" int tcavt_transpose_ct(const float* in, float* out_f32, void* out_bf16, int B, int C, int To,
                                  int dtype16, tcavt_stream_t stream) {
  TCAVT_CHECK_ARG(in && (out_f32 || out_bf16) && B > 0 && C > 0 && To > 0, "transpose_ct: bad args");
  TCAVT_CHECK_ARG(is16(dtype16), "transpose_ct: dtype16 must be TCAVT_BF16 or TCAVT_F16");
  const long n = (long)B * C * To;
  hipLaunchKernelGGL(transpose_ct_kernel, dim3((unsigned)((n + 255) / 256)), dim3(256), 0,
                     static_cast<hipStream_t>(stream), in, out_f32, static_cast<bf16_t*>(out_bf16), B, C, To,
                     dtype16 == TCAVT_F16 ? 1 : 0);
  TCAVT_CHECK_LAUNCH("transpose_ct");
  return TCAVT_OK;
}

extern "C" int tcavt_out_head(const float* fused, const float* w, const float* bias, const float* x,
                              float* out, int B, int To, int C, int F, int T, int add_last,
                              tcavt_stream_t stream) {
  TCAVT_CHECK_ARG(fused && w && bias && x && out && B > 0 && To > 0 && C > 0 && F > 0 && T > 0,
                  "out_head: bad args");
  const int n = B * F * To;
  hipLaunchKernelGGL(out_head_kernel, dim3((n + 255) / 256), dim3(256), 0, static_cast<hipStream_t>(stream),
                     fused, w, bias, x, out, B, To, C, F, T, add_last);
  TCAVT_CHECK_LAUNCH("out_head");
  return TCAVT_OK;
}

extern "C" int tcavt_traj_metrics(const float* pred, const float* gt, const float* norm_stat,
                                  float* sums, int32_t* argmin, float* per_sample, int B, int K, int To,
                                  tcavt_stream_t stream) {
  TCAVT_CHECK_ARG(pred && gt && norm_stat && sums && B > 0 && K > 0 && To > 0, "traj_metrics: bad args");
  hipLaunchKernelGGL(traj_metrics_kernel, dim3(1), dim3(1024), 0, static_cast<hipStream_t>(stream), pred, gt,
                     norm_stat, sums, argmin, per_sample, B, K, To);
  TCAVT_CHECK_LAUNCH("traj_metrics");
  return TCAVT_OK;
}
```

### traffic-context-augmented-vehicle-trajectory-prediction-framework-using-multimodal-llm_amd/csrc/tlayers.hip

```cpp
#include "common.hpp"

using namespace tcavt;

#define TCAVT_TRY(call)            \
  do {                             \
    const int rc_ = (call);        \
    if (rc_ != TCAVT_OK) return rc_; \
  } while (0)

namespace {
struct Ctx {
  const tcavt_tstack_args* a;
  tcavt_stream_t st;
  uint32_t site;
  int M;

  int gemm(const void* A16, const float* A32, const void* W, const float* bias, void* C, int out_dtype, int Mr, int N, int K,
           bool relu, const float* residual, bool drop) {
    const float p = drop ? a->dropout_p : 0.f;
    const uint32_t s = drop && a->dropout_p > 0.f ? site++ : 0u;
    int flags = (bias ? TCAVT_EPI_BIAS : 0) | (relu ? TCAVT_EPI_RELU : 0) | (residual ? TCAVT_EPI_RESIDUAL : 0);
    if (a->dtype16) {
      tcavt_gemm_args g = {};
      g.A = A16; g.lda = K; g.W = W; g.ldw = K; g.C = C; g.ldc = N; g.M = Mr; g.N = N; g.K = K;
      g.out_dtype = out_dtype; g.in_dtype = a->dtype16; g.epilogue = flags; g.bias = bias; g.residual = residual; g.ldr = N;
      g.dropout_p = p; g.dropout_seed = a->dropout_seed; g.dropout_site = s;
      return tcavt_gemm_bf16(&g, st);
    }
    return tcavt_gemm_f32(A32, K, static_cast<const float*>(W), K, bias, residual, N, static_cast<float*>(C), N, Mr, N, K, flags, p,
                          a->dropout_seed, s, st);
  }
  int norm(const float* y, const float* w, const float* b, float* out, void* outb) {
    return tcavt_layernorm(y, nullptr, w, b, 1e-5f, out, a->dtype16 ? outb : nullptr, M, a->E, a->dtype16 ? a->dtype16 : TCAVT_BF16, st);
  }
};
}

extern "C" int tcavt_tlayer_stack_forward(const tcavt_tstack_args* a, tcavt_stream_t stream) {
  TCAVT_CHECK_ARG(a && a->layers && a->n_layers > 0 && a->x && a->B > 0 && a->L > 0 && a->E > 0 && a->FF > 0 && a->nhead > 0 &&
                      a->E % a->nhead == 0,
                  "tlayer_stack_forward: bad args");
  TCAVT_CHECK_ARG(a->dtype16 == 0 || is16(a->dtype16), "tlayer_stack_forward: dtype16 must be 0 (fp32 layers), TCAVT_BF16 or TCAVT_F16");
  TCAVT_CHECK_ARG(!a->dtype16 || a->xb, "tlayer_stack_forward: 16-bit layers need the 16-bit copy of the input tokens");
  TCAVT_CHECK_ARG(a->dropout_p >= 0.f && a->dropout_p < 1.f, "tlayer_stack_forward: dropout_p must be in [0, 1)");
  const int E = a->E, FF = a->FF, nh = a->nhead, dh = E / nh, M = a->B * a->L;
  const int act = a->dtype16 ? a->dtype16 : TCAVT_F32;
  const float scale = (float)(1.0 / sqrt((double)dh));
  Ctx c{a, stream, a->first_site, M};
  auto mha_site = [&]() -> uint32_t { return a->dropout_p > 0.f ? c.site++ : 0u; };
  const float* x = a->x;
  const void* xb = a->xb;
  for (int li = 0; li < a->n_layers; ++li) {
    const tcavt_tlayer& l = a->layers[li];
    const bool dec = l.w_q != nullptr;
    TCAVT_CHECK_ARG(l.w_in && l.b_in && l.w_out && l.b_out && l.w1 && l.b1 && l.w2 && l.b2 && l.n1_w && l.n1_b && l.n2_w && l.n2_b &&
                        l.qkv && l.att && l.y && l.x1 && l.ffh && l.y2 && l.out && (!a->dtype16 || (l.x1b && l.outb)),
                    "tlayer_stack_forward: layer %d: null weight / buffer", li);
    if (dec)
      TCAVT_CHECK_ARG(a->mem && (!a->dtype16 || a->memb) && a->Lk > 0 && l.b_q && l.w_kv && l.b_kv && l.w_co && l.b_co && l.n3_w &&
                          l.n3_b && l.cq && l.ckv && l.catt && l.cy && l.x2 && (!a->dtype16 || l.x2b),
                      "tlayer_stack_forward: layer %d: decoder layer without memory / cross-attention buffers", li);
    TCAVT_TRY(c.gemm(xb, x, l.w_in, l.b_in, l.qkv, TCAVT_F32, M, 3 * E, E, false, nullptr, false));
    {
      const uint32_t s = mha_site();
      TCAVT_TRY(tcavt_mha(l.qkv, 3 * E, l.qkv + E, 3 * E, l.qkv + 2 * E, 3 * E, l.att, E, a->key_len, a->B, a->L, a->L, nh, dh, scale,
                          TCAVT_F32, act, a->dropout_p, a->dropout_seed, s, stream));
    }
    TCAVT_TRY(c.gemm(l.att, static_cast<const float*>(l.att), l.w_out, l.b_out, l.y, TCAVT_F32, M, E, E, false, x, true));
    TCAVT_TRY(c.norm(l.y, l.n1_w, l.n1_b, l.x1, l.x1b));
    const float* xin = l.x1;
    const void* xinb = l.x1b;
    if (dec) {
      const int Mk = a->B * a->Lk;
      TCAVT_TRY(c.gemm(l.x1b, l.x1, l.w_q, l.b_q, l.cq, TCAVT_F32, M, E, E, false, nullptr, false));
      TCAVT_TRY(c.gemm(a->memb, a->mem, l.w_kv, l.b_kv, l.ckv, TCAVT_F32, Mk, 2 * E, E, false, nullptr, false));
      const uint32_t s = mha_site();
      TCAVT_TRY(tcavt_mha(l.cq, E, l.ckv, 2 * E, l.ckv + E, 2 * E, l.catt, E, nullptr, a->B, a->L, a->Lk, nh, dh, scale, TCAVT_F32, act,
                          a->dropout_p, a->dropout_seed, s, stream));
      TCAVT_TRY(c.gemm(l.catt, static_cast<const float*>(l.catt), l.w_co, l.b_co, l.cy, TCAVT_F32, M, E, E, false, l.x1, true));
      TCAVT_TRY(c.norm(l.cy, l.n2_w, l.n2_b, l.x2, l.x2b));
      xin = l.x2;
      xinb = l.x2b;
    }
    TCAVT_TRY(c.gemm(xinb, xin, l.w1, l.b1, l.ffh, act, M, FF, E, true, nullptr, true));
    TCAVT_TRY(c.gemm(l.ffh, static_cast<const float*>(l.ffh), l.w2, l.b2, l.y2, TCAVT_F32, M, E, FF, false, xin, true));
    TCAVT_TRY(c.norm(l.y2, dec ? l.n3_w : l.n2_w, dec ? l.n3_b : l.n2_b, l.out, l.outb));
    x = l.out;
    xb = l.outb;
  }
  return TCAVT_OK;
}

extern "C" int tcavt_tlayer_stack_backward(const tcavt_tstack_bwd_args* a, tcavt_stream_t stream) {
  TCAVT_CHECK_ARG(a && a->fwd && a->grads && a->g_out && a->g_x && a->g_tmp && a->g_y2 && a->g_x1 && a->g_y && a->g_att && a->g_f &&
                      a->g_qkv,
                  "tlayer_stack_backward: null pointer");
  const tcavt_tstack_args& f = *a->fwd;
  TCAVT_CHECK_ARG(f.layers && f.n_layers > 0 && f.x && f.B > 0 && f.L > 0 && f.E > 0 && f.FF > 0 && f.nhead > 0 && f.E % f.nhead == 0,
                  "tlayer_stack_backward: bad forward args");
  TCAVT_CHECK_ARG(f.dtype16 == 0, "tlayer_stack_backward: fp32 layers only (the 16-bit stacks' backward is composed by the caller)");
  TCAVT_CHECK_ARG(f.dropout_p >= 0.f && f.dropout_p < 1.f && (f.dropout_p == 0.f || (a->g_y2d && a->g_yd)),
                  "tlayer_stack_backward: dropout_p in [0, 1); train mode needs g_y2d / g_yd");
  const int E = f.E, FF = f.FF, nh = f.nhead, dh = E / nh, M = f.B * f.L;
  const float p = f.dropout_p;
  const float scale = (float)(1.0 / sqrt((double)dh));
  auto lin32 = [&](const float* x, const float* W, const float* gy, float* gW, float* gb, float* gx, int Mr, int N, int K) -> int {
    TCAVT_TRY(tcavt_gemm_f32_strided(gy, 1, N, x, 1, K, nullptr, nullptr, 0, gW, K, N, K, Mr, TCAVT_EPI_ACCUM, a->red_ws, a->red_ws_elems, stream));
    TCAVT_TRY(tcavt_colsum(gy, N, TCAVT_F32, gb, Mr, N, 1, a->red_ws, a->red_ws_elems, stream));
    return tcavt_gemm_f32_strided(gy, N, 1, W, 1, K, nullptr, nullptr, 0, gx, K, Mr, K, N, 0, a->red_ws, a->red_ws_elems, stream);
  };
  const float* g_in = a->g_out;
  for (int li = f.n_layers - 1; li >= 0; --li) {
    const tcavt_tlayer& l = f.layers[li];
    const tcavt_tlayer_grads& g = a->grads[li];
    TCAVT_CHECK_ARG(!l.w_q, "tlayer_stack_backward: layer %d is a decoder layer (encoder layers only)", li);
    TCAVT_CHECK_ARG(l.w_in && l.w_out && l.w1 && l.w2 && l.n1_w && l.n2_w && l.qkv && l.att && l.y && l.x1 && l.ffh && l.y2 &&
                        (li == 0 || f.layers[li - 1].out) && g.g_w_in && g.g_b_in && g.g_w_out && g.g_b_out && g.g_w1 && g.g_b1 &&
                        g.g_w2 && g.g_b2 && g.g_n1_w && g.g_n1_b && g.g_n2_w && g.g_n2_b,
                    "tlayer_stack_backward: layer %d: null weight / activation / gradient", li);
    const float* x_in = li == 0 ? f.x : f.layers[li - 1].out;
    const uint32_t s = f.first_site + 4u * (uint32_t)li;
    float* g_xin = (li & 1) ? a->g_tmp : a->g_x;
    auto drop = [&](const float* gi, float* go, int64_t n, uint32_t site) {
      return tcavt_dropout(gi, go, n, TCAVT_F32, p, f.dropout_seed, site, nullptr, stream);
    };
    TCAVT_TRY(tcavt_layernorm_bwd(l.y2, l.n2_w, g_in, 1e-5f, a->g_y2, g.g_n2_w, g.g_n2_b, M, E, a->red_ws, a->red_ws_elems, stream));
    const float* g_y2d = a->g_y2;
    if (p > 0.f) {
      TCAVT_TRY(drop(a->g_y2, a->g_y2d, (int64_t)M * E, s + 3));
      g_y2d = a->g_y2d;
    }
    const float* ffh = static_cast<const float*>(l.ffh);
    TCAVT_TRY(lin32(ffh, static_cast<const float*>(l.w2), g_y2d, g.g_w2, g.g_b2, a->g_f, M, E, FF));
    if (p > 0.f) TCAVT_TRY(drop(a->g_f, a->g_f, (int64_t)M * FF, s + 2));
    TCAVT_TRY(tcavt_relu_bwd(a->g_f, ffh, TCAVT_F32, (int64_t)M * FF, stream));
    TCAVT_TRY(lin32(l.x1, static_cast<const float*>(l.w1), a->g_f, g.g_w1, g.g_b1, a->g_x1, M, FF, E));
    TCAVT_TRY(tcavt_add_inplace(a->g_x1, a->g_y2, (int64_t)M * E, stream));
    TCAVT_TRY(tcavt_layernorm_bwd(l.y, l.n1_w, a->g_x1, 1e-5f, a->g_y, g.g_n1_w, g.g_n1_b, M, E, a->red_ws, a->red_ws_elems, stream));
    const float* g_yd = a->g_y;
    if (p > 0.f) {
      TCAVT_TRY(drop(a->g_y, a->g_yd, (int64_t)M * E, s + 1));
      g_yd = a->g_yd;
    }
    TCAVT_TRY(lin32(static_cast<const float*>(l.att), static_cast<const float*>(l.w_out), g_yd, g.g_w_out, g.g_b_out, a->g_att, M, E, E));
    TCAVT_TRY(tcavt_mha_bwd(l.qkv, 3 * E, l.qkv + E, 3 * E, l.qkv + 2 * E, 3 * E, a->g_att, E, a->g_qkv, a->g_qkv + E, a->g_qkv + 2 * E,
                            3 * E, f.key_len, f.B, f.L, f.L, nh, dh, scale, p, f.dropout_seed, p > 0.f ? s : 0u, stream));
    TCAVT_TRY(lin32(x_in, static_cast<const float*>(l.w_in), a->g_qkv, g.g_w_in, g.g_b_in, g_xin, M, 3 * E, E));
    TCAVT_TRY(tcavt_add_inplace(g_xin, a->g_y, (int64_t)M * E, stream));
    g_in = g_xin;
  }
  return TCAVT_OK;
}

extern "C" int tcavt_cross_attn_forward(const tcavt_cross_attn_args* a, tcavt_stream_t stream) {
  TCAVT_CHECK_ARG(a && a->q && a->wk_t && a->w_v && a->b_v && a->fh && a->fh_t && a->qp && a->scores && a->probs && a->ctx && a->att,
                  "cross_attn_forward: null pointer");
  TCAVT_CHECK_ARG(a->B > 0 && a->To > 0 && a->L > 0 && a->Lp >= a->L && a->Lp % 64 == 0 && a->H > 0 && a->nhead > 0 &&
                      a->H % a->nhead == 0 && (a->H / a->nhead) % 64 == 0 && a->H % 64 == 0,
                  "cross_attn_forward: bad shape (Lp %% 64 == 0 >= L, head dim %% 64 == 0)");
  TCAVT_CHECK_ARG(a->dtype16 == TCAVT_F16, "cross_attn_forward: fp16 storage only (the probabilities are carried in fp16)");
  TCAVT_CHECK_ARG(a->dropout_p >= 0.f && a->dropout_p < 1.f, "cross_attn_forward: dropout_p must be in [0, 1)");
  const int B = a->B, To = a->To, L = a->L, Lp = a->Lp, H = a->H, nh = a->nhead, dh = H / nh, M = B * To, dt = a->dtype16;
  const char* q = static_cast<const char*>(a->q);
  const char* wk_t = static_cast<const char*>(a->wk_t);
  const char* w_v = static_cast<const char*>(a->w_v);
  char* qp = static_cast<char*>(a->qp);
  char* ctx = static_cast<char*>(a->ctx);
  char* att = static_cast<char*>(a->att);
  TCAVT_TRY(tcavt_transpose16(a->fh, H, a->fh_t, (int64_t)B * Lp, L, H, Lp, B, (int64_t)L * H, Lp, 0, stream));
  for (int h = 0; h < nh; ++h) {
    tcavt_gemm_args g = {};
    g.A = q + (size_t)h * dh * 2; g.lda = H; g.W = wk_t + (size_t)h * H * dh * 2; g.ldw = dh;
    g.C = qp + (size_t)h * M * H * 2; g.ldc = H; g.M = M; g.N = H; g.K = dh; g.out_dtype = dt; g.in_dtype = dt;
    TCAVT_TRY(tcavt_gemm_bf16(&g, stream));
  }
  {
    tcavt_gemm_args g = {};
    g.A = a->qp; g.lda = H; g.W = a->fh; g.ldw = H; g.C = a->scores; g.ldc = Lp; g.M = To; g.N = Lp; g.K = H;
    g.out_dtype = TCAVT_F32; g.in_dtype = dt; g.tile = 64; g.acc_scale = (float)(1.0 / sqrt((double)dh));
    g.batch = B * nh; g.batch_inner = nh;
    g.sAo = (int64_t)To * H; g.sAi = (int64_t)M * H; g.sWo = (int64_t)L * H; g.sWi = 0;
    g.sCo = (int64_t)nh * To * Lp; g.sCi = (int64_t)To * Lp;
    TCAVT_TRY(tcavt_gemm_bf16(&g, stream));
  }
  TCAVT_TRY(tcavt_softmax_rows(a->scores, Lp, a->probs, Lp, TCAVT_F16, B * nh * To, L, Lp, a->dropout_p, a->dropout_seed,
                               a->dropout_site, stream));
  {
    tcavt_gemm_args g = {};
    g.A = a->probs; g.lda = Lp; g.W = a->fh_t; g.ldw = (int64_t)B * Lp; g.C = a->ctx; g.ldc = H; g.M = To; g.N = H; g.K = Lp;
    g.out_dtype = dt; g.in_dtype = TCAVT_F16; g.tile = 64;
    g.batch = B * nh; g.batch_inner = nh;
// ... 2 lines not shown
    TCAVT_TRY(tcavt_gemm_bf16(&g, stream));
  }
  for (int h = 0; h < nh; ++h) {
    tcavt_gemm_args g = {};
    g.A = ctx + (size_t)h * M * H * 2; g.lda = H; g.W = w_v + (size_t)h * dh * H * 2; g.ldw = H;
    g.C = att + (size_t)h * dh * 2; g.ldc = H; g.M = M; g.N = dh; g.K = H; g.out_dtype = dt; g.in_dtype = dt;
    g.bias = a->b_v + (size_t)h * dh; g.epilogue = TCAVT_EPI_BIAS;
    TCAVT_TRY(tcavt_gemm_bf16(&g, stream));
  }
  return TCAVT_OK;
}

extern "C" int tcavt_ltsf_forward(const tcavt_ltsf_args* a, int phase, tcavt_stream_t stream) {
  TCAVT_CHECK_ARG(a && (phase == 1 || phase == 2 || phase == 3), "ltsf_forward: phase must be 1 (front), 2 (head) or 3 (both)");
  TCAVT_CHECK_ARG(a->B > 0 && a->C > 0 && a->T > 0 && a->To > 0 && a->F > 0 && a->nhead_sa > 0 && a->C % a->nhead_sa == 0,
                  "ltsf_forward: bad shape");
  TCAVT_CHECK_ARG(a->dropout_p >= 0.f && a->dropout_p < 1.f, "ltsf_forward: dropout_p must be in [0, 1)");
  const int B = a->B, C = a->C, T = a->T, To = a->To, Mt = B * T, Mo = B * To;
  const float p = a->dropout_p;
  const uint64_t seed = a->dropout_seed;
  const uint32_t s0 = a->first_site;
  auto gf32 = [&](const float* A, const float* W, const float* bias, float* Cc, int M, int N, int K, bool relu, const float* res,
                  int site_off) {
    const int flags = (bias ? TCAVT_EPI_BIAS : 0) | (relu ? TCAVT_EPI_RELU : 0) | (res ? TCAVT_EPI_RESIDUAL : 0);
    const bool drop = site_off >= 0 && p > 0.f;
    return tcavt_gemm_f32(A, K, W, K, bias, res, N, Cc, N, M, N, K, flags, drop ? p : 0.f, seed, drop ? s0 + (uint32_t)site_off : 0u,
                          stream);
  };
  if (phase & 1) {
    TCAVT_CHECK_ARG(a->x && a->conv_w && a->conv_b && a->enc_w && a->enc_b && a->pos && a->tok && a->sa_n1_w && a->sa_n1_b &&
                        a->sa_in_w && a->sa_in_b && a->sa_out_w && a->sa_out_b && a->sa_n2_w && a->sa_n2_b && a->sa_f0_w &&
                        a->sa_f0_b && a->sa_f3_w && a->sa_f3_b && a->sa_xn && a->sa_qkv && a->sa_att && a->sa_res1 && a->sa_rn &&
                        a->sa_f && a->e,
                    "ltsf_forward: phase 1: null pointer");
    TCAVT_TRY(tcavt_ltsf_front(a->x, a->conv_w, a->conv_b, a->enc_w, a->enc_b, a->pos, a->tok, a->xp_tok, B, C, T, stream));
    const int dh = C / a->nhead_sa;
    TCAVT_TRY(tcavt_layernorm(a->tok, nullptr, a->sa_n1_w, a->sa_n1_b, 1e-5f, a->sa_xn, nullptr, Mt, C, TCAVT_BF16, stream));
    TCAVT_TRY(gf32(a->sa_xn, a->sa_in_w, a->sa_in_b, a->sa_qkv, Mt, 3 * C, C, false, nullptr, -1));
    TCAVT_TRY(tcavt_mha(a->sa_qkv, 3 * C, a->sa_qkv + C, 3 * C, a->sa_qkv + 2 * C, 3 * C, a->sa_att, C, nullptr, B, T, T, a->nhead_sa,
                        dh, (float)(1.0 / sqrt((double)dh)), TCAVT_F32, TCAVT_F32, p, seed, p > 0.f ? s0 : 0u, stream));
    TCAVT_TRY(gf32(a->sa_att, a->sa_out_w, a->sa_out_b, a->sa_res1, Mt, C, C, false, a->sa_xn, 1));
    TCAVT_TRY(tcavt_layernorm(a->sa_res1, nullptr, a->sa_n2_w, a->sa_n2_b, 1e-5f, a->sa_rn, nullptr, Mt, C, TCAVT_BF16, stream));
    TCAVT_TRY(gf32(a->sa_rn, a->sa_f0_w, a->sa_f0_b, a->sa_f, Mt, 4 * C, C, true, nullptr, 2));
    TCAVT_TRY(gf32(a->sa_f, a->sa_f3_w, a->sa_f3_b, a->e, Mt, C, 4 * C, false, a->sa_rn, 3));
  }
  if (phase & 2) {
    TCAVT_CHECK_ARG(a->e && a->poly_emb && a->lane_w && a->lane_b && a->dec_w && a->dec_b && a->lane && a->d0 && a->dec_t &&
                        a->dec_tb && a->w_dp && a->b_dp && a->proj && a->w_q && a->b_q && a->xattn.q && a->w_co && a->b_co &&
                        a->cross && a->w_un && a->b_un && a->fused && a->fl_n_w && a->fl_n_b && a->fn && a->fl1_w && a->fl1_b &&
                        a->f1 && a->fl3_w && a->fl3_b && a->f2 && a->out_w && a->out_b && a->x && a->out && a->poly_dim > 0 &&
                        a->H > 0,
                    "ltsf_forward: phase 2: null pointer");
    const int H = a->H, CT = C * To;
    TCAVT_TRY(gf32(a->poly_emb, a->lane_w, a->lane_b, a->lane, B, CT, a->poly_dim, false, nullptr, -1));
    TCAVT_TRY(tcavt_ltsf_decode(a->e, a->dec_w, a->dec_b, a->lane, a->d0, B, C, T, To, stream));
    const float* d1 = a->d0;
    if (a->post_hidden > 0) {
      TCAVT_CHECK_ARG(a->pm0_w && a->pm0_b && a->pm3_w && a->pm3_b && a->hid && a->d1, "ltsf_forward: post-MLP: null pointer");
      TCAVT_TRY(gf32(a->d0, a->pm0_w, a->pm0_b, a->hid, B, a->post_hidden, CT, true, nullptr, 4));
      TCAVT_TRY(gf32(a->hid, a->pm3_w, a->pm3_b, a->d1, B, CT, a->post_hidden, false, nullptr, -1));
      d1 = a->d1;
    }
    TCAVT_TRY(tcavt_transpose_ct(d1, a->dec_t, a->dec_tb, B, C, To, TCAVT_F16, stream));
    auto g16 = [&](const void* A, const void* W, const float* bias, void* Cc, int out_dtype, int M, int N, int K, const float* res) {
      tcavt_gemm_args g = {};
      g.A = A; g.lda = K; g.W = W; g.ldw = K; g.C = Cc; g.ldc = N; g.M = M; g.N = N; g.K = K; g.out_dtype = out_dtype;
      g.in_dtype = TCAVT_F16; g.bias = bias; g.residual = res; g.ldr = N;
      g.epilogue = (bias ? TCAVT_EPI_BIAS : 0) | (res ? TCAVT_EPI_RESIDUAL : 0);
      return tcavt_gemm_bf16(&g, stream);
    };
    TCAVT_TRY(g16(a->dec_tb, a->w_dp, a->b_dp, a->proj, TCAVT_F16, Mo, H, C, nullptr));
    TCAVT_TRY(g16(a->proj, a->w_q, a->b_q, const_cast<void*>(a->xattn.q), TCAVT_F16, Mo, H, H, nullptr));
    TCAVT_TRY(tcavt_cross_attn_forward(&a->xattn, stream));
    TCAVT_TRY(g16(a->xattn.att, a->w_co, a->b_co, a->cross, TCAVT_F16, Mo, H, H, nullptr));
    TCAVT_TRY(g16(a->cross, a->w_un, a->b_un, a->fused, TCAVT_F32, Mo, C, H, a->dec_t));
    TCAVT_TRY(tcavt_layernorm(a->fused, nullptr, a->fl_n_w, a->fl_n_b, 1e-5f, a->fn, nullptr, Mo, C, TCAVT_BF16, stream));
    TCAVT_TRY(gf32(a->fn, a->fl1_w, a->fl1_b, a->f1, Mo, C, C, true, nullptr, -1));
    TCAVT_TRY(gf32(a->f1, a->fl3_w, a->fl3_b, a->f2, Mo, C, C, false, nullptr, -1));
    TCAVT_TRY(tcavt_out_head(a->f2, a->out_w, a->out_b, a->x, a->out, B, To, C, a->F, T, a->add_last, stream));
  }
  return TCAVT_OK;
}

extern "C" int tcavt_cross_attn_backward(const tcavt_cross_attn_bwd_args* a, tcavt_stream_t stream) {
  TCAVT_CHECK_ARG(a && a->fwd && a->g_att && a->w_in && a->gw_in && a->gb_in && a->g_q && a->fh_tb && a->fh_b && a->ga_t &&
                      a->g_ctx && a->w_t && a->x_t && a->d_p && a->d_s && a->g_qp,
                  "cross_attn_backward: null pointer");
  const tcavt_cross_attn_args& f = *a->fwd;
  const int B = f.B, To = f.To, L = f.L, Lp = f.Lp, H = f.H, nh = f.nhead, dh = H / nh, M = B * To, Mp = (M + 63) / 64 * 64;
  TCAVT_CHECK_ARG(f.dtype16 == TCAVT_F16 && (f.dropout_p == 0.f || a->p_undropped), "cross_attn_backward: fp16 forward; train mode needs p_undropped");
  const float scale = (float)(1.0 / sqrt((double)dh));
  const int BF = TCAVT_BF16;
  char* g_att = static_cast<char*>(const_cast<void*>(a->g_att));
  char* g_ctx = static_cast<char*>(a->g_ctx);
  char* g_qp = static_cast<char*>(a->g_qp);
  char* g_q = static_cast<char*>(a->g_q);
  char* ga_t = static_cast<char*>(a->ga_t);
  const char* ctx = static_cast<const char*>(f.ctx);
  const char* q = static_cast<const char*>(f.q);
  auto gemm = [&](const void* A, int64_t lda, const void* W, int64_t ldw, void* C, int64_t ldc, int out_dtype, int Mr, int N, int K) {
    tcavt_gemm_args g = {};
    g.A = A; g.lda = lda; g.W = W; g.ldw = ldw; g.C = C; g.ldc = ldc; g.M = Mr; g.N = N; g.K = K; g.out_dtype = out_dtype; g.in_dtype = BF;
    return tcavt_gemm_bf16(&g, stream);
  };
  TCAVT_TRY(tcavt_transpose16(f.fh, H, a->fh_tb, (int64_t)B * Lp, L, H, Lp, B, (int64_t)L * H, Lp, 1, stream));
  TCAVT_TRY(tcavt_transpose16(a->fh_tb, (int64_t)B * Lp, a->fh_b, H, H, B * Lp, H, 1, 0, 0, 0, stream));
  TCAVT_TRY(tcavt_colsum(a->g_att, H, BF, a->gb_in + 2 * H, M, H, 1, a->red_ws, a->red_ws_elems, stream));
  TCAVT_TRY(tcavt_transpose16(a->g_att, H, a->ga_t, Mp, M, H, Mp, 1, 0, 0, 0, stream));
  for (int h = 0; h < nh; ++h) {
    const float* Wv_h = a->w_in + (size_t)(2 * H + h * dh) * H;
    TCAVT_TRY(tcavt_transpose_f32_bf16(Wv_h, H, a->w_t, dh, dh, H, dh, stream));
    TCAVT_TRY(gemm(g_att + (size_t)h * dh * 2, H, a->w_t, dh, g_ctx + (size_t)h * M * H * 2, H, BF, M, H, dh));
    TCAVT_TRY(tcavt_transpose16(ctx + (size_t)h * M * H * 2, H, a->x_t, Mp, M, H, Mp, 1, 0, 0, 1, stream));
    TCAVT_TRY(gemm(ga_t + (size_t)h * dh * Mp * 2, Mp, a->x_t, Mp, a->gw_in + (size_t)(2 * H + h * dh) * H, H, TCAVT_F32, dh, H, Mp));
  }
  {
    tcavt_gemm_args g = {};
    g.A = a->g_ctx; g.lda = H; g.W = a->fh_b; g.ldw = H; g.C = a->d_p; g.ldc = Lp; g.M = To; g.N = Lp; g.K = H;
    g.out_dtype = TCAVT_F32; g.in_dtype = BF; g.tile = 64; g.batch = B * nh; g.batch_inner = nh;
    g.sAo = (int64_t)To * H; g.sAi = (int64_t)M * H; g.sWo = (int64_t)Lp * H; g.sWi = 0;
    g.sCo = (int64_t)nh * To * Lp; g.sCi = (int64_t)To * Lp;
    TCAVT_TRY(tcavt_gemm_bf16(&g, stream));
  }
  const void* p_used = f.probs;
  if (f.dropout_p > 0.f) {
    TCAVT_TRY(tcavt_dropout(a->d_p, a->d_p, (int64_t)B * nh * To * Lp, TCAVT_F32, f.dropout_p, f.dropout_seed, f.dropout_site, nullptr, stream));
    TCAVT_TRY(tcavt_softmax_rows(f.scores, Lp, a->p_undropped, Lp, TCAVT_F16, B * nh * To, L, Lp, 0.f, 0, 0, stream));
    p_used = a->p_undropped;
  }
  TCAVT_TRY(tcavt_softmax_bwd_rows(p_used, Lp, a->d_p, Lp, a->d_s, Lp, scale, B * nh * To, L, Lp, stream));
  {
    tcavt_gemm_args g = {};
    g.A = a->d_s; g.lda = Lp; g.W = a->fh_tb; g.ldw = (int64_t)B * Lp; g.C = a->g_qp; g.ldc = H; g.M = To; g.N = H; g.K = Lp;
    g.out_dtype = BF; g.in_dtype = BF; g.tile = 64; g.batch = B * nh; g.batch_inner = nh;
    g.sAo = (int64_t)nh * To * Lp; g.sAi = (int64_t)To * Lp; g.sWo = Lp; g.sWi = 0;
    g.sCo = (int64_t)To * H; g.sCi = (int64_t)M * H;
    TCAVT_TRY(tcavt_gemm_bf16(&g, stream));
  }
  for (int h = 0; h < nh; ++h) {
    const float* Wk_h = a->w_in + (size_t)(H + h * dh) * H;
    TCAVT_TRY(tcavt_cast_f32_16(Wk_h, a->w_t, (int64_t)dh * H, BF, stream));
    TCAVT_TRY(gemm(g_qp + (size_t)h * M * H * 2, H, a->w_t, H, g_q + (size_t)h * dh * 2, H, BF, M, dh, H));
    TCAVT_TRY(tcavt_transpose16(q + (size_t)h * dh * 2, H, a->ga_t, Mp, M, dh, Mp, 1, 0, 0, 1, stream));
    TCAVT_TRY(tcavt_transpose16(g_qp + (size_t)h * M * H * 2, H, a->x_t, Mp, M, H, Mp, 1, 0, 0, 0, stream));
    TCAVT_TRY(gemm(a->ga_t, Mp, a->x_t, Mp, a->gw_in + (size_t)(H + h * dh) * H, H, TCAVT_F32, dh, H, Mp));
  }
  return TCAVT_OK;
}

namespace {
__global__ __launch_bounds__(256) void copy_rows_kernel(const float* __restrict__ src, long ld_src, float* __restrict__ dst,
                                                        long ld_dst, int width) {
  const float* s = src + (long)blockIdx.x * ld_src;
  float* d = dst + (long)blockIdx.x * ld_dst;
  for (int i = threadIdx.x; i < width; i += 256) d[i] = s[i];
}

int copy_rows(const float* src, long ld_src, float* dst, long ld_dst, int rows, int width, tcavt_stream_t stream) {
  hipLaunchKernelGGL(copy_rows_kernel, dim3(rows), dim3(256), 0, static_cast<hipStream_t>(stream), src, ld_src, dst, ld_dst, width);
  TCAVT_CHECK_LAUNCH("ltsf_backward: copy_rows");
  return TCAVT_OK;
}
}

extern "C" int tcavt_ltsf_backward(const tcavt_ltsf_bwd_args* a, int phase, tcavt_stream_t stream) {
  TCAVT_CHECK_ARG(a && a->fwd && (phase == 1 || phase == 2 || phase == 3), "ltsf_backward: phase must be 1 (head), 2 (front) or 3 (both)");
  const tcavt_ltsf_args& f = *a->fwd;
  TCAVT_CHECK_ARG(f.B > 0 && f.C > 0 && f.T > 0 && f.To > 0 && f.F > 0 && f.H > 0 && f.nhead_sa > 0 && f.C % f.nhead_sa == 0 &&
                      f.poly_dim > 0,
                  "ltsf_backward: bad shape");
  TCAVT_CHECK_ARG(f.dropout_p >= 0.f && f.dropout_p < 1.f, "ltsf_backward: dropout_p must be in [0, 1)");
  const int B = f.B, C = f.C, T = f.T, To = f.To, H = f.H, Mo = B * To, Mt = B * T, CT = C * To, Mp = (Mo + 63) / 64 * 64;
  const float p = f.dropout_p;
  const uint64_t seed = f.dropout_seed;
  const uint32_t s0 = f.first_site;
  const int BF = TCAVT_BF16;
  auto lin32 = [&](const float* x, const float* W, const float* gy, float* gW, float* gb, float* gx, int M, int N, int K) -> int {
    TCAVT_TRY(tcavt_gemm_f32_strided(gy, 1, N, x, 1, K, nullptr, nullptr, 0, gW, K, N, K, M, TCAVT_EPI_ACCUM, a->red_ws, a->red_ws_elems, stream));
    TCAVT_TRY(tcavt_colsum(gy, N, TCAVT_F32, gb, M, N, 1, a->red_ws, a->red_ws_elems, stream));
    if (gx) TCAVT_TRY(tcavt_gemm_f32_strided(gy, N, 1, W, 1, K, nullptr, nullptr, 0, gx, K, M, K, N, 0, a->red_ws, a->red_ws_elems, stream));
    return TCAVT_OK;
  };
  auto lin16 = [&](const void* x16, const float* W, const void* gy, int gy_dtype, float* gW, float* gb, void* gx, int gx_dtype,
                   int N, int K) -> int {
    const void* gyb = gy;
    if (gy_dtype == TCAVT_F32) {
      TCAVT_TRY(tcavt_cast_f32_16(static_cast<const float*>(gy), a->s_gyb, (int64_t)Mo * N, BF, stream));
      gyb = a->s_gyb;
    }
    TCAVT_TRY(tcavt_transpose16(gyb, N, a->s_gyt, Mp, Mo, N, Mp, 1, 0, 0, 0, stream));
    TCAVT_TRY(tcavt_transpose16(x16, K, a->s_xt, Mp, Mo, K, Mp, 1, 0, 0, 1, stream));
    tcavt_gemm_args g = {};
    g.A = a->s_gyt; g.lda = Mp; g.W = a->s_xt; g.ldw = Mp; g.C = gW; g.ldc = K; g.M = N; g.N = K; g.K = Mp;
    g.out_dtype = TCAVT_F32; g.in_dtype = BF;
    TCAVT_TRY(tcavt_gemm_bf16(&g, stream));
    TCAVT_TRY(tcavt_colsum(gy, N, gy_dtype, gb, Mo, N, 1, a->red_ws, a->red_ws_elems, stream));
    TCAVT_TRY(tcavt_transpose_f32_bf16(W, K, a->s_wt, N, N, K, N, stream));
    tcavt_gemm_args d = {};
    d.A = gyb; d.lda = N; d.W = a->s_wt; d.ldw = N; d.C = gx; d.ldc = K; d.M = Mo; d.N = K; d.K = N;
    d.out_dtype = gx_dtype; d.in_dtype = BF;
    return tcavt_gemm_bf16(&d, stream);
  };
  auto drop = [&](const float* g, float* out, int64_t n, int site_off) -> int {
    return tcavt_dropout(g, out, n, TCAVT_F32, p, seed, s0 + (uint32_t)site_off, nullptr, stream);
  };

  if (phase & 1) {
    TCAVT_CHECK_ARG(a->g_out && f.f2 && f.f1 && f.fn && f.fused && f.cross && f.xattn.att && f.xattn.q && f.proj && f.dec_tb && f.d0 &&
                        f.poly_emb && f.out_w && f.fl3_w && f.fl1_w && f.fl_n_w && f.lane_w && a->w_un && a->w_co && a->w_dp &&
                        a->xattn.w_in && a->xattn.gw_in && a->xattn.gb_in && a->xattn.g_att && a->xattn.g_q,
                    "ltsf_backward: phase 1: null forward pointer");
    TCAVT_CHECK_ARG(a->g_out_w && a->g_out_b && a->g_fl3_w && a->g_fl3_b && a->g_fl1_w && a->g_fl1_b && a->g_fl_n_w && a->g_fl_n_b &&
                        a->g_un_w && a->g_un_b && a->g_co_w && a->g_co_b && a->g_dp_w && a->g_dp_b && a->g_lane_w && a->g_lane_b &&
                        a->g_poly && a->g_f2 && a->g_f1 && a->g_fn && a->g_dec_t && a->g_dt2 && a->g_cross && a->g_proj && a->g_d1 &&
                        a->s_gyb && a->s_gyt && a->s_xt && a->s_wt,
                    "ltsf_backward: phase 1: null gradient pointer / workspace");
    TCAVT_CHECK_ARG(a->xattn.fwd == &f.xattn, "ltsf_backward: xattn.fwd must point at fwd->xattn");
    TCAVT_TRY(tcavt_out_head_bwd(a->g_out, f.f2, f.out_w, a->g_f2, a->g_out_w, a->g_out_b, B, To, C, f.F, stream));
    TCAVT_TRY(lin32(f.f1, f.fl3_w, a->g_f2, a->g_fl3_w, a->g_fl3_b, a->g_f1, Mo, C, C));
    TCAVT_TRY(tcavt_relu_bwd(a->g_f1, f.f1, TCAVT_F32, (int64_t)Mo * C, stream));
    TCAVT_TRY(lin32(f.fn, f.fl1_w, a->g_f1, a->g_fl1_w, a->g_fl1_b, a->g_fn, Mo, C, C));
    TCAVT_TRY(tcavt_layernorm_bwd(f.fused, f.fl_n_w, a->g_fn, 1e-5f, a->g_dec_t, a->g_fl_n_w, a->g_fl_n_b, Mo, C, a->red_ws, a->red_ws_elems, stream));
    TCAVT_TRY(lin16(f.cross, a->w_un, a->g_dec_t, TCAVT_F32, a->g_un_w, a->g_un_b, a->g_cross, BF, C, H));
    TCAVT_TRY(lin16(f.xattn.att, a->w_co, a->g_cross, BF, a->g_co_w, a->g_co_b, const_cast<void*>(a->xattn.g_att), BF, H, H));
    TCAVT_TRY(tcavt_cross_attn_backward(&a->xattn, stream));
    TCAVT_TRY(lin16(f.proj, a->xattn.w_in, a->xattn.g_q, BF, a->xattn.gw_in, a->xattn.gb_in, a->g_proj, BF, H, H));
    TCAVT_TRY(lin16(f.dec_tb, a->w_dp, a->g_proj, BF, a->g_dp_w, a->g_dp_b, a->g_dt2, TCAVT_F32, H, C));
    TCAVT_TRY(tcavt_add_inplace(a->g_dt2, a->g_dec_t, (int64_t)Mo * C, stream));
    TCAVT_TRY(tcavt_transpose_ct(a->g_dt2, a->g_d1, nullptr, B, To, C, BF, stream));
    const float* g_d0 = a->g_d1;
    if (f.post_hidden > 0) {
      TCAVT_CHECK_ARG(f.hid && f.pm0_w && f.pm3_w && a->g_hid && a->g_d0 && a->g_pm0_w && a->g_pm0_b && a->g_pm3_w && a->g_pm3_b,
                      "ltsf_backward: post-MLP: null pointer");
      TCAVT_TRY(lin32(f.hid, f.pm3_w, a->g_d1, a->g_pm3_w, a->g_pm3_b, a->g_hid, B, CT, f.post_hidden));
      if (p > 0.f) TCAVT_TRY(drop(a->g_hid, a->g_hid, (int64_t)B * f.post_hidden, 4));
      TCAVT_TRY(tcavt_relu_bwd(a->g_hid, f.hid, TCAVT_F32, (int64_t)B * f.post_hidden, stream));
      TCAVT_TRY(lin32(f.d0, f.pm0_w, a->g_hid, a->g_pm0_w, a->g_pm0_b, a->g_d0, B, f.post_hidden, CT));
      g_d0 = a->g_d0;
    }
    TCAVT_TRY(lin32(f.poly_emb, f.lane_w, g_d0, a->g_lane_w, a->g_lane_b, a->g_poly, B, CT, f.poly_dim));
  }
  if (phase & 2) {
    TCAVT_CHECK_ARG(f.e && f.dec_w && f.enc_w && f.tok && f.xp_tok && f.x && f.sa_xn && f.sa_qkv && f.sa_att && f.sa_res1 && f.sa_rn &&
                        f.sa_f && f.sa_n1_w && f.sa_in_w && f.sa_out_w && f.sa_n2_w && f.sa_f0_w && f.sa_f3_w,
                    "ltsf_backward: phase 2: null forward pointer (the forward must keep xp_tok)");
    TCAVT_CHECK_ARG(a->g_dec_w && a->g_dec_b && a->g_enc_w && a->g_enc_b && a->g_pos && a->pos_ld >= T && a->g_conv_w && a->g_conv_b &&
                        a->g_sa_n1_w && a->g_sa_n1_b && a->g_sa_in_w && a->g_sa_in_b && a->g_sa_out_w && a->g_sa_out_b && a->g_sa_n2_w &&
                        a->g_sa_n2_b && a->g_sa_f0_w && a->g_sa_f0_b && a->g_sa_f3_w && a->g_sa_f3_b && a->g_dw && a->g_db && a->g_e &&
                        a->g_ff && a->g_rn && a->g_res1 && a->g_att_sa && a->g_qkv && a->g_xn && a->g_tok && a->g_ew && a->g_eb &&
                        a->g_xp && (p == 0.f || (a->g_e_d && a->g_res1_d)) && (f.post_hidden > 0 ? a->g_d0 != nullptr : a->g_d1 != nullptr),
                    "ltsf_backward: phase 2: null gradient pointer / workspace");
    const float* g_d0 = f.post_hidden > 0 ? a->g_d0 : a->g_d1;
    TCAVT_TRY(tcavt_nlinear_bwd(f.e, f.dec_w, g_d0, CT, To, 1, a->g_dw, a->g_db, a->g_e, B, C, T, To, stream));
    TCAVT_TRY(copy_rows(a->g_dw, (long)To * T, a->g_dec_w, a->dec_stride, C, To * T, stream));
    TCAVT_TRY(copy_rows(a->g_db, To, a->g_dec_b, a->dec_stride, C, To, stream));
    const float* g_e_d = a->g_e;
    if (p > 0.f) {
      TCAVT_TRY(drop(a->g_e, a->g_e_d, (int64_t)Mt * C, 3));
      g_e_d = a->g_e_d;
    }
    TCAVT_TRY(lin32(f.sa_f, f.sa_f3_w, g_e_d, a->g_sa_f3_w, a->g_sa_f3_b, a->g_ff, Mt, C, 4 * C));
    if (p > 0.f) TCAVT_TRY(drop(a->g_ff, a->g_ff, (int64_t)Mt * 4 * C, 2));
    TCAVT_TRY(tcavt_relu_bwd(a->g_ff, f.sa_f, TCAVT_F32, (int64_t)Mt * 4 * C, stream));
    TCAVT_TRY(lin32(f.sa_rn, f.sa_f0_w, a->g_ff, a->g_sa_f0_w, a->g_sa_f0_b, a->g_rn, Mt, 4 * C, C));
    TCAVT_TRY(tcavt_add_inplace(a->g_rn, a->g_e, (int64_t)Mt * C, stream));
    TCAVT_TRY(tcavt_layernorm_bwd(f.sa_res1, f.sa_n2_w, a->g_rn, 1e-5f, a->g_res1, a->g_sa_n2_w, a->g_sa_n2_b, Mt, C, a->red_ws, a->red_ws_elems, stream));
    const float* g_res1_d = a->g_res1;
    if (p > 0.f) {
      TCAVT_TRY(drop(a->g_res1, a->g_res1_d, (int64_t)Mt * C, 1));
      g_res1_d = a->g_res1_d;
    }
    TCAVT_TRY(lin32(f.sa_att, f.sa_out_w, g_res1_d, a->g_sa_out_w, a->g_sa_out_b, a->g_att_sa, Mt, C, C));
    const int dh = C / f.nhead_sa;
    TCAVT_TRY(tcavt_mha_bwd(f.sa_qkv, 3 * C, f.sa_qkv + C, 3 * C, f.sa_qkv + 2 * C, 3 * C, a->g_att_sa, C, a->g_qkv, a->g_qkv + C,
                            a->g_qkv + 2 * C, 3 * C, nullptr, B, T, T, f.nhead_sa, dh, (float)(1.0 / sqrt((double)dh)), p, seed,
                            p > 0.f ? s0 : 0u, stream));
    TCAVT_TRY(lin32(f.sa_xn, f.sa_in_w, a->g_qkv, a->g_sa_in_w, a->g_sa_in_b, a->g_xn, Mt, 3 * C, C));
    TCAVT_TRY(tcavt_add_inplace(a->g_xn, a->g_res1, (int64_t)Mt * C, stream));
    TCAVT_TRY(tcavt_layernorm_bwd(f.tok, f.sa_n1_w, a->g_xn, 1e-5f, a->g_tok, a->g_sa_n1_w, a->g_sa_n1_b, Mt, C, a->red_ws, a->red_ws_elems, stream));
    TCAVT_TRY(tcavt_nlinear_bwd(f.xp_tok, f.enc_w, a->g_tok, (int64_t)T * C, 1, C, a->g_ew, a->g_eb, a->g_xp, B, C, T, T, stream));
    TCAVT_TRY(copy_rows(a->g_ew, (long)T * T, a->g_enc_w, a->enc_stride, C, T * T, stream));
    TCAVT_TRY(copy_rows(a->g_eb, T, a->g_enc_b, a->enc_stride, C, T, stream));
    TCAVT_TRY(copy_rows(a->g_eb, T, a->g_pos, a->pos_ld, C, T, stream));
    TCAVT_TRY(tcavt_conv1x1_bwd(a->g_xp, f.x, a->g_conv_w, a->g_conv_b, B, C, T, f.F, stream));
  }
  return TCAVT_OK;
}
```

### traffic-context-augmented-vehicle-trajectory-prediction-framework-using-multimodal-llm_amd/ops.py

```python
import ctypes

import torch

from . import capi
from .capi import BF16, EPI_BIAS, EPI_RELU, EPI_RESIDUAL, EPI_ROPE, EPI_SILU_MUL, F32, check, lib, ptr, stream_ptr

__all__ = [
    "gemm_bf16", "rmsnorm", "layernorm", "cast_bf16", "embed_fuse", "mask_to_kvlen", "attn_causal_gqa", "mha", "gemm_f32",
    "poly_embed", "masked_mean", "ltsf_front", "ltsf_decode", "transpose_ct", "out_head", "traj_metrics",
]


_ALLOW_CPU = False


def _req(t, dtype, name):
    if t is None:
        return
    if not t.is_cuda and not _ALLOW_CPU:
        raise capi.TcavtError(f"{name}: tensor must live on the GPU (no CPU fallback)")
    if t.dtype != dtype:
        raise capi.TcavtError(f"{name}: expected {dtype}, got {t.dtype}")
    if not t.is_contiguous():
        raise capi.TcavtError(f"{name}: tensor must be contiguous")
# ... 692 lines not shown
                                       stream_ptr()), "tcavt_softmax_bwd_rows")


def mse_grad(pred, gt, norm_stat, g, B, To):
    for t, n, nm in ((pred, B * 2 * To, "pred"), (gt, B * 2 * To, "gt"), (norm_stat, B * 4, "norm_stat"), (g, B * 2 * To, "g")):
        _req(t, torch.float32, "mse_grad." + nm)
        _need(t, n, "mse_grad." + nm)
    check(lib().tcavt_mse_grad(ptr(pred), ptr(gt), ptr(norm_stat), ptr(g), B, To, stream_ptr()), "tcavt_mse_grad")


def mse_grad_seeded(pred, gt, norm_stat, g, B, To, g_loss=None, g_pred=None):
    if g_loss is None and g_pred is None:
        raise capi.TcavtError("mse_grad_seeded: g_loss and g_pred are both None")
    checks = [(g, B * 2 * To, "g"), (g_loss, 1, "g_loss"), (g_pred, B * 2 * To, "g_pred")]
    if g_loss is not None:
        checks += [(pred, B * 2 * To, "pred"), (gt, B * 2 * To, "gt"), (norm_stat, B * 4, "norm_stat")]
    for t, n, nm in checks:
        _req(t, torch.float32, "mse_grad_seeded." + nm)
        _need(t, n, "mse_grad_seeded." + nm)
    if g_loss is None:
        pred = gt = norm_stat = None
    check(lib().tcavt_mse_grad_seeded(ptr(pred), ptr(gt), ptr(norm_stat), ptr(g_loss), ptr(g_pred), ptr(g), B, To,
                                      stream_ptr()), "tcavt_mse_grad_seeded")


def out_head_bwd(g, fused, w, gf, gw, gb, B, To, C, F):
    for t, n, nm in ((g, B * F * To, "g"), (fused, B * To * C, "fused"), (w, F * C, "w"), (gf, B * To * C, "gf"),
                     (gw, F * C, "gw"), (gb, F, "gb")):
        _need(t, n, "out_head_bwd." + nm)
    check(lib().tcavt_out_head_bwd(ptr(g), ptr(fused), ptr(w), ptr(gf), ptr(gw), ptr(gb), B, To, C, F, stream_ptr()),
          "tcavt_out_head_bwd")


def nlinear_bwd(in_tok, W, g, g_strides, gW, gbias, gin_tok, B, C, T, S):
    sb, sc, ss = g_strides
    for t, n, nm in ((in_tok, B * T * C, "in_tok"), (W, C * S * T, "W"), (gW, C * S * T, "gW"), (gbias, C * S, "gbias"),
                     (gin_tok, B * T * C, "gin_tok")):
        _need(t, n, "nlinear_bwd." + nm)
    if _avail(g) < (B - 1) * sb + (C - 1) * sc + (S - 1) * ss + 1:
        raise capi.TcavtError("nlinear_bwd.g: buffer too small")
    check(lib().tcavt_nlinear_bwd(ptr(in_tok), ptr(W), ptr(g), sb, sc, ss, ptr(gW), ptr(gbias), ptr(gin_tok), B, C, T, S,
                                  stream_ptr()), "tcavt_nlinear_bwd")


def conv1x1_bwd(gxp_tok, x, gw, gb, B, C, T, F):
    for t, n, nm in ((gxp_tok, B * T * C, "gxp_tok"), (x, B * F * T, "x"), (gw, C * F, "gw"), (gb, C, "gb")):
        _need(t, n, "conv1x1_bwd." + nm)
    check(lib().tcavt_conv1x1_bwd(ptr(gxp_tok), ptr(x), ptr(gw), ptr(gb), B, C, T, F, stream_ptr()), "tcavt_conv1x1_bwd")


def poly_embed_bwd(g, polygon, gw, gb, gpos, B, P, D):
    for t, n, nm in ((g, B * P * D, "g"), (polygon, B * P * 2, "polygon"), (gw, D * 2, "gw"), (gb, D, "gb"), (gpos, P * D, "gpos")):
        _need(t, n, "poly_embed_bwd." + nm)
    check(lib().tcavt_poly_embed_bwd(ptr(g), ptr(polygon), ptr(gw), ptr(gb), ptr(gpos), B, P, D, stream_ptr()),
          "tcavt_poly_embed_bwd")


def masked_mean_bwd(gemb, lens, genc, B, P, D):
    for t, n, nm in ((gemb, B * D, "gemb"), (lens, B, "lens"), (genc, B * P * D, "genc")):
        _need(t, n, "masked_mean_bwd." + nm)
    check(lib().tcavt_masked_mean_bwd(ptr(gemb), ptr(lens), ptr(genc), B, P, D, stream_ptr()), "tcavt_masked_mean_bwd")


def wgrad_tn(g, g_col0, n, x, out, trans_out=False, rs_part=None, rs_h=0, rs_eps=0.0):
    if g.dtype not in _H16 or x.dtype not in _H16 or out.dtype != torch.float32 or (g.dtype == torch.float16 and x.dtype != torch.float16):
        raise capi.TcavtError("wgrad_tn: g bf16 with x fp16 / bf16, or g fp16 with x fp16; out fp32")
    M, H = x.shape
    if g.shape[0] < M or g.shape[1] < g_col0 + n or g.stride(1) != 1 or x.stride(1) != 1 or out.stride(1) != 1:
        raise capi.TcavtError("wgrad_tn: operand shapes / strides")
    rows, cols = (H, n) if trans_out else (n, H)
    if out.shape[0] < rows or out.shape[1] < cols:
        raise capi.TcavtError(f"wgrad_tn.out: needs at least ({rows}, {cols})")
    npart = 0
    if rs_part is not None:
        _req(rs_part, torch.float32, "wgrad_tn.rs_part")
        if rs_part.dim() != 2 or rs_part.shape[0] < M or not rs_part.is_contiguous() or rs_h <= 0:
            raise capi.TcavtError("wgrad_tn.rs_part: contiguous fp32 [M, npart] and rs_h > 0 required")
        npart = rs_part.shape[1]
    check(lib().tcavt_wgrad_tn(ptr(g), g.stride(0), int(g_col0), int(n), ptr(x), x.stride(0), _DT[x.dtype], ptr(out), out.stride(0),
                               M, H, int(trans_out), _DT[g.dtype], ptr(rs_part) if rs_part is not None else None, npart, int(rs_h),
                               float(rs_eps), stream_ptr()), "tcavt_wgrad_tn")


def lora_wgrad_a(x16, part, gamma, g_t, dA, eps, dropout=None, site_v=None):
    _req16(x16, "lora_wgrad_a.x16")
    _req16(g_t, "lora_wgrad_a.g_t", like=x16)
    _req(part, torch.float32, "lora_wgrad_a.part")
    _req(gamma, torch.float32, "lora_wgrad_a.gamma")
    _req(dA, torch.float32, "lora_wgrad_a.dA")
    M, H = x16.shape
    if (part.dim() != 2 or part.shape[0] < M or not part.is_contiguous() or g_t.shape[0] < M or g_t.shape[1] != 64
            or not g_t.is_contiguous() or dA.dim() != 2 or dA.shape[0] < 32 or dA.shape[1] < H or dA.stride(1) != 1):
        raise capi.TcavtError("lora_wgrad_a: part [M, npart], g_t [M, 64], dA [>= 32, >= H] required")
    _need(gamma, H, "lora_wgrad_a.gamma")
    p, seed, site = _drop(dropout)
    check(lib().tcavt_lora_wgrad_a(ptr(x16), ptr(part), part.shape[1], float(eps), ptr(gamma), ptr(g_t), ptr(dA), dA.stride(0), M, H,
                                   p, seed, site, site + 1 if site_v is None else int(site_v), _DT16(x16), stream_ptr()),
          "tcavt_lora_wgrad_a")


def clip_grad_norm(g, max_norm, scratch, grad_scale=1.0):
    _req(g, torch.float32, "clip_grad_norm.g")
    _req(scratch, torch.float32, "clip_grad_norm.scratch")
    _need(scratch, 1026, "clip_grad_norm.scratch")
    check(lib().tcavt_clip_grad_norm(ptr(g), g.numel(), float(max_norm), float(grad_scale), ptr(scratch), stream_ptr()),
          "tcavt_clip_grad_norm")


def adamw(p, g, m, v, lr, beta1, beta2, eps, weight_decay, step, grad_scale=1.0):
    n = p.numel()
    for t, nm in ((p, "p"), (g, "g"), (m, "m"), (v, "v")):
        _req(t, torch.float32, "adamw." + nm)
        _need(t, n, "adamw." + nm)
    check(lib().tcavt_adamw(ptr(p), ptr(g), ptr(m), ptr(v), n, lr, beta1, beta2, eps, weight_decay, int(step),
                            grad_scale, stream_ptr()), "tcavt_adamw")


def adamw_gated(p, g, m, v, lr, beta1, beta2, eps, weight_decay, loss, ctl, grad_scale=1.0, grad_norm=None):
    n = p.numel()
    for t, nm in ((p, "p"), (g, "g"), (m, "m"), (v, "v")):
        _req(t, torch.float32, "adamw_gated." + nm)
        _need(t, n, "adamw_gated." + nm)
    _req(loss, torch.float32, "adamw_gated.loss")
    _need(loss, 1, "adamw_gated.loss")
    _req(ctl, torch.int32, "adamw_gated.ctl")
    _need(ctl, 8, "adamw_gated.ctl")
    if grad_norm is not None:
        _req(grad_norm, torch.float32, "adamw_gated.grad_norm")
        _need(grad_norm, 1, "adamw_gated.grad_norm")
    check(lib().tcavt_adamw_gated(ptr(p), ptr(g), ptr(m), ptr(v), n, lr, beta1, beta2, eps, weight_decay, grad_scale,
                                  ptr(loss), ptr(grad_norm), ptr(ctl), stream_ptr()), "tcavt_adamw_gated")


def llama_stack_forward(args):
    check(lib().tcavt_llama_stack_forward(ctypes.byref(args), stream_ptr()), "tcavt_llama_stack_forward")


def lora_down(x16, a_cat, t, scale, dropout=None, site_v=None):
    _req16(x16, "lora_down.x16")
    _req16(a_cat, "lora_down.a_cat", like=x16)
    _req16(t, "lora_down.t", like=x16)
    M, H = x16.shape
    _need(a_cat, 32 * H, "lora_down.a_cat")
    _need(t, M * 64, "lora_down.t")
    p, seed, site = _drop(dropout)
    check(lib().tcavt_lora_down(ptr(x16), ptr(a_cat), ptr(t), M, H, float(scale), p, seed, site,
                                (site + 1) if site_v is None else int(site_v), _DT[x16.dtype], stream_ptr()), "tcavt_lora_down")


def lora_dgrad(g_t, a_qT, a_vT, out, dropout=None, site_v=None):
    _req16(g_t, "lora_dgrad.g_t")
    for t, nm in ((a_qT, "a_qT"), (a_vT, "a_vT"), (out, "out")):
        _req16(t, "lora_dgrad." + nm, like=g_t)
    M, H = out.shape
    _need(g_t, M * 64, "lora_dgrad.g_t")
    _need(a_qT, H * 64, "lora_dgrad.a_qT")
    _need(a_vT, H * 64, "lora_dgrad.a_vT")
    p, seed, site = _drop(dropout)
    check(lib().tcavt_lora_dgrad(ptr(g_t), ptr(a_qT), ptr(a_vT), ptr(out), M, H, p, seed, site,
                                 (site + 1) if site_v is None else int(site_v), _DT[g_t.dtype], stream_ptr()), "tcavt_lora_dgrad")


def copy_batch(dsts, srcs):
    n = len(dsts)
    if n != len(srcs) or not 0 < n <= 16:
        raise capi.TcavtError("copy_batch: 1 .. 16 (dst, src) pairs")
# ... 244 lines not shown
```

Baseline: 2207.

## Add transpose-free TN/NN GEMM kernels with fused bias column sums in backward

Adds a gemm_tn kernel that reads row-major G and X directly, transposing tiles in LDS and accumulating bias sums on the fly. It also adds a batched gemm_nn path and an f32 strided GEMM with a fused rowsum. Together these replace the separate transpose16 passes, padded staging buffers and colsum launches in the LTSF and cross-attention backward. The aim is fewer kernel launches and less global traffic. The cost is a new hand-written kernel with software prefetch whose tile efficiency may be lower than the existing GEMM.

```diff
diff --git a/include/tcavt.h b/include/tcavt.h
--- a/include/tcavt.h
+++ b/include/tcavt.h
@@ -164,6 +164,10 @@
                            int64_t ldc, int M, int N, int K, int flags, float* ws, int64_t ws_elems,
                            tcavt_stream_t stream);
 
+int tcavt_gemm_f32_strided_rowsum(const float* A, int64_t rsA, int64_t csA, const float* W, int64_t rsW, int64_t csW,
+                                  float* C, int64_t ldc, int M, int N, int K, int flags, float* rowsum,
+                                  int rowsum_accumulate, float* ws, int64_t ws_elems, tcavt_stream_t stream);
+
 
 int tcavt_transpose16(const void* in, int64_t ld_in, void* out, int64_t ld_out, int rows, int cols,
                       int rows_pad, int batch, int64_t s_in, int64_t s_out, int f16_to_bf16, tcavt_stream_t stream);
@@ -207,6 +211,19 @@
 int tcavt_wgrad_tn(const void* G, int64_t ldg, int g_col0, int n, const void* X, int64_t ldx, int x_dtype, float* C,
                    int64_t ldc, int M, int H, int trans_out, int g_dtype, const float* rs_part, int rs_npart, int rs_h,
                    float rs_eps, tcavt_stream_t stream);
+int tcavt_gemm_tn(const void* G, int64_t ldg, int g_col0, int g_dtype, const void* X, int64_t ldx, int x_dtype, float* C,
+                  int64_t ldc, int N, int H, int M, float* gb, int gb_accumulate, tcavt_stream_t stream);
+typedef struct tcavt_gemm_nn_args {
+  const void* A;
+  const void* X;
+  void* C;
+  int64_t lda, ldx, ldc;
+  int M, N, K;
+  int a_dtype, x_dtype, out_dtype;
+  int batch, batch_inner;
+  int64_t sAo, sAi, sXo, sXi, sCo, sCi;
+} tcavt_gemm_nn_args;
+int tcavt_gemm_nn(const tcavt_gemm_nn_args* a, tcavt_stream_t stream);
 int tcavt_lora_wgrad_a(const void* x16, const float* part, int npart, float eps, const float* gamma, const void* g_t, float* dA,
                        int64_t ldc, int M, int H, float dropout_p, uint64_t dropout_seed, uint32_t site_q, uint32_t site_v,
                        int dtype16, tcavt_stream_t stream);
diff --git a/traffic-context-augmented-vehicle-trajectory-prediction-framework-using-multimodal-llm_amd/capi.py b/traffic-context-augmented-vehicle-trajectory-prediction-framework-using-multimodal-llm_amd/capi.py
--- a/traffic-context-augmented-vehicle-trajectory-prediction-framework-using-multimodal-llm_amd/capi.py
+++ b/traffic-context-augmented-vehicle-trajectory-prediction-framework-using-multimodal-llm_amd/capi.py
@@ -14,6 +14,14 @@
 W_FRAG16 = 1
 
 c_void_p, c_int, c_int64, c_float = ctypes.c_void_p, ctypes.c_int, ctypes.c_int64, ctypes.c_float
+
+
+class GemmNnArgs(ctypes.Structure):
+
+    _fields_ = [("A", c_void_p), ("X", c_void_p), ("C", c_void_p), ("lda", c_int64), ("ldx", c_int64), ("ldc", c_int64),
+                ("M", c_int), ("N", c_int), ("K", c_int), ("a_dtype", c_int), ("x_dtype", c_int), ("out_dtype", c_int),
+                ("batch", c_int), ("batch_inner", c_int), ("sAo", c_int64), ("sAi", c_int64), ("sXo", c_int64), ("sXi", c_int64),
+                ("sCo", c_int64), ("sCi", c_int64)]
 
 
 class GemmArgs(ctypes.Structure):
@@ -242,6 +250,8 @@
                            c_void_p],
     "tcavt_gemm_f32_strided": [c_void_p, c_int64, c_int64, c_void_p, c_int64, c_int64, c_void_p, c_void_p, c_int64,
                                c_void_p, c_int64, c_int, c_int, c_int, c_int, c_void_p, c_int64, c_void_p],
+    "tcavt_gemm_f32_strided_rowsum": [c_void_p, c_int64, c_int64, c_void_p, c_int64, c_int64, c_void_p, c_int64, c_int, c_int, c_int,
+                                      c_int, c_void_p, c_int, c_void_p, c_int64, c_void_p],
     "tcavt_transpose16": [c_void_p, c_int64, c_void_p, c_int64, c_int, c_int, c_int, c_int, c_int64, c_int64, c_int, c_void_p],
     "tcavt_transpose_f32_bf16": [c_void_p, c_int64, c_void_p, c_int64, c_int, c_int, c_int, c_void_p],
     "tcavt_colsum": [c_void_p, c_int64, c_int, c_void_p, c_int, c_int, c_int, c_void_p, c_int64, c_void_p],
@@ -273,6 +283,9 @@
     "tcavt_gqa_rope_bwd_pack": [c_void_p, c_void_p, c_void_p, c_void_p, c_int64, c_int, c_int, c_int, c_int, c_void_p],
     "tcavt_wgrad_tn": [c_void_p, c_int64, c_int, c_int, c_void_p, c_int64, c_int, c_void_p, c_int64, c_int, c_int, c_int, c_int,
                        c_void_p, c_int, c_int, c_float, c_void_p],
+    "tcavt_gemm_tn": [c_void_p, c_int64, c_int, c_int, c_void_p, c_int64, c_int, c_void_p, c_int64, c_int, c_int, c_int, c_void_p,
+                      c_int, c_void_p],
+    "tcavt_gemm_nn": [ctypes.POINTER(GemmNnArgs), c_void_p],
     "tcavt_lora_wgrad_a": [c_void_p, c_void_p, c_int, c_float, c_void_p, c_void_p, c_void_p, c_int64, c_int, c_int, c_float,
                            ctypes.c_uint64, ctypes.c_uint32, ctypes.c_uint32, c_int, c_void_p],
     "tcavt_clip_grad_norm": [c_void_p, c_int64, c_float, c_float, c_void_p, c_void_p],
diff --git a/traffic-context-augmented-vehicle-trajectory-prediction-framework-using-multimodal-llm_amd/csrc/llm_backward.hip b/traffic-context-augmented-vehicle-trajectory-prediction-framework-using-multimodal-llm_amd/csrc/llm_backward.hip
--- a/traffic-context-augmented-vehicle-trajectory-prediction-framework-using-multimodal-llm_amd/csrc/llm_backward.hip
+++ b/traffic-context-augmented-vehicle-trajectory-prediction-framework-using-multimodal-llm_amd/csrc/llm_backward.hip
@@ -1530,13 +1530,39 @@
     }
 }
 
+constexpr int kTnXS = 40;
+__device__ __forceinline__ void tn_store8(bf16_t* __restrict__ t, int col, int row, const u32x4& v) {
+#pragma unroll
+  for (int e = 0; e < 4; ++e) {
+    t[(col + 2 * e) * kTnXS + row] = static_cast<bf16_t>(v[e] & 0xffffu);
+    t[(col + 2 * e + 1) * kTnXS + row] = static_cast<bf16_t>(v[e] >> 16);
+  }
+}
+template <bool GF16>
+__device__ __forceinline__ void tn_mma(const bf16_t* __restrict__ xt, const bf16_t* __restrict__ gt, int NB, f32x4 (&acc)[4][4], int wave,
+                                       int r16, int kq) {
+  u32x4 bf[4];
+#pragma unroll
+  for (int b = 0; b < 4; ++b) bf[b] = *reinterpret_cast<const u32x4*>(&xt[(wave * 64 + b * 16 + r16) * kTnXS + kq * 8]);
+#pragma unroll
+  for (int a = 0; a < 4; ++a) {
+    if (a < NB) {
+      const u32x4 af = *reinterpret_cast<const u32x4*>(&gt[(a * 16 + r16) * kTnXS + kq * 8]);
+#pragma unroll
+      for (int b = 0; b < 4; ++b)
+        acc[a][b] = mfma16b<GF16>(__builtin_bit_cast(bf16x8, af), __builtin_bit_cast(bf16x8, bf[b]), acc[a][b]);
+    }
+  }
+}
+__device__ __forceinline__ unsigned int f16x2_to_bf16x2(unsigned int w) { return pack_bf16x2(from16_lo<true>(w), from16_hi<true>(w)); }
+
 template <bool XF16, bool GF16 = false>
 __global__ __launch_bounds__(256) void wgrad_tn_kernel(const bf16_t* __restrict__ G, long ldg, int g0, int NB,
                                                        const bf16_t* __restrict__ X, long ldx, float* __restrict__ C,
                                                        long ldc, int M, int H, int m_per_wg, int trans_out,
                                                        const float* __restrict__ rs_part, int rs_npart, float rs_inv_h,
                                                        float rs_eps) {
-  constexpr int XS = 40;
+  constexpr int XS = kTnXS;
   __shared__ __attribute__((aligned(16))) bf16_t xt[256 * XS];
   __shared__ __attribute__((aligned(16))) bf16_t gt[64 * XS];
   const int tid = threadIdx.x, lane = tid & 63, wave = tid >> 6;
@@ -1559,16 +1585,11 @@
         u32x4 v = {0u, 0u, 0u, 0u};
         const int col = h0 + xc0 + c * 8;
         if (ok && col < H) v = *reinterpret_cast<const u32x4*>(X + (long)m * ldx + col);
-#pragma unroll
-        for (int e = 0; e < 4; ++e) {
-          bf16_t lo = static_cast<bf16_t>(v[e] & 0xffffu), hi = static_cast<bf16_t>(v[e] >> 16);
-          if constexpr (XF16 && !GF16) {
-            lo = f32_to_bf16(f16_to_f32(lo));
-            hi = f32_to_bf16(f16_to_f32(hi));
-          }
-          xt[(xc0 + c * 8 + 2 * e) * XS + xrow] = lo;
-          xt[(xc0 + c * 8 + 2 * e + 1) * XS + xrow] = hi;
-        }
+        if constexpr (XF16 && !GF16) {
+#pragma unroll
+          for (int e = 0; e < 4; ++e) v[e] = f16x2_to_bf16x2(v[e]);
+        }
+        tn_store8(xt, xc0 + c * 8, xrow, v);
       }
       if (gc0 < 16 * NB) {
         u32x4 v = {0u, 0u, 0u, 0u};
@@ -1579,26 +1600,11 @@
 #pragma unroll
           for (int e = 0; e < 4; ++e) v[e] = pack16x2<GF16>(from16_lo<GF16>(v[e]) * rs, from16_hi<GF16>(v[e]) * rs);
         }
-#pragma unroll
-        for (int e = 0; e < 4; ++e) {
-          gt[(gc0 + 2 * e) * XS + grow] = static_cast<bf16_t>(v[e] & 0xffffu);
-          gt[(gc0 + 2 * e + 1) * XS + grow] = static_cast<bf16_t>(v[e] >> 16);
-        }
+        tn_store8(gt, gc0, grow, v);
       }
     }
     __syncthreads();
-    u32x4 bf[4];
-#pragma unroll
-    for (int b = 0; b < 4; ++b) bf[b] = *reinterpret_cast<const u32x4*>(&xt[(wave * 64 + b * 16 + r16) * XS + kq * 8]);
-#pragma unroll
-    for (int a = 0; a < 4; ++a) {
-      if (a < NB) {
-        const u32x4 af = *reinterpret_cast<const u32x4*>(&gt[(a * 16 + r16) * XS + kq * 8]);
-#pragma unroll
-        for (int b = 0; b < 4; ++b)
-          acc[a][b] = mfma16b<GF16>(__builtin_bit_cast(bf16x8, af), __builtin_bit_cast(bf16x8, bf[b]), acc[a][b]);
-      }
-    }
+    tn_mma<GF16>(xt, gt, NB, acc, wave, r16, kq);
     __syncthreads();
   }
 #pragma unroll
@@ -1614,6 +1620,147 @@
         float* dst = trans_out ? C + (long)h * ldc + n : C + (long)n * ldc + h;
         atomicAdd(dst, acc[a][b][e]);
       }
+    }
+  }
+}
+
+__device__ __forceinline__ u32x4 tn_load8(const bf16_t* __restrict__ row, int col, int ncols, bool ok) {
+  u32x4 v = {0u, 0u, 0u, 0u};
+  if (ok && col + 8 <= ncols) {
+    v = *reinterpret_cast<const u32x4*>(row + col);
+  } else if (ok) {
+#pragma unroll
+    for (int e = 0; e < 8; ++e)
+      if (col + e < ncols) v[e >> 1] |= static_cast<unsigned int>(row[col + e]) << (16 * (e & 1));
+  }
+  return v;
+}
+
+struct TnP {
+  const void* G;
+  const bf16_t* X;
+  void* C;
+  float* gb;
+  long ldg, ldx, ldc;
+  int g0, N, M, H, gb_acc, out_kind, batch_inner;
+  long sGo, sGi, sXo, sXi, sCo, sCi;
+};
+
+template <bool XF16, int GT, bool GC = false>
+__global__ __launch_bounds__(256) void gemm_tn_kernel(TnP p) {
+  constexpr bool GF16 = GT == 1;
+  static_assert(GT != 1 || XF16, "the f16 MFMA takes both operands in fp16");
+  static_assert(!GC || GT != 2, "the contraction-contiguous first operand is 16-bit");
+  __shared__ __attribute__((aligned(16))) bf16_t xt[256 * kTnXS];
+  __shared__ __attribute__((aligned(16))) bf16_t gt[64 * kTnXS];
+  const int tid = threadIdx.x, lane = tid & 63, wave = tid >> 6;
+  const int h0 = blockIdx.x * 256, i0 = blockIdx.y * 64;
+  const int bo = blockIdx.z / p.batch_inner, bi = blockIdx.z - bo * p.batch_inner;
+  const long goff = bo * p.sGo + bi * p.sGi, coff = bo * p.sCo + bi * p.sCi;
+  const void* Gv = GT == 2 ? static_cast<const void*>(static_cast<const float*>(p.G) + goff)
+                           : static_cast<const void*>(static_cast<const bf16_t*>(p.G) + goff);
+  const bf16_t* X = p.X + bo * p.sXo + bi * p.sXi;
+  const long ldg = p.ldg, ldx = p.ldx, ldc = p.ldc;
+  const int g0 = p.g0, N = p.N, M = p.M, H = p.H, gb_acc = p.gb_acc;
+  float* gb = p.gb;
+  const int r16 = lane & 15, kq = lane >> 4;
+  const int NB = min(4, (N - i0 + 15) >> 4);
+  f32x4 acc[4][4];
+#pragma unroll
+  for (int a = 0; a < 4; ++a)
+#pragma unroll
+    for (int b = 0; b < 4; ++b) acc[a][b] = f32x4{0.f, 0.f, 0.f, 0.f};
+  const int xrow = tid >> 3, xc0 = (tid & 7) * 32;
+  const int gc0 = (tid & 7) * 8;
+  const bool want_b = gb != nullptr && blockIdx.x == 0;
+  float bsum[8];
+#pragma unroll
+  for (int e = 0; e < 8; ++e) bsum[e] = 0.f;
+  u32x4 xv[4], gv;
+  auto load = [&](int m0) {
+    const int m = m0 + xrow;
+    const bool ok = m < M;
+    const bf16_t* xr = X + (long)m * ldx;
+#pragma unroll
+    for (int c = 0; c < 4; ++c) {
+      xv[c] = tn_load8(xr, h0 + xc0 + c * 8, H, ok);
+      if constexpr (XF16 && !GF16) {
+#pragma unroll
+        for (int e = 0; e < 4; ++e) xv[c][e] = f16x2_to_bf16x2(xv[c][e]);
+      }
+    }
+    const int col = i0 + gc0;
+    if constexpr (GC) {
+      const int i = i0 + (tid >> 2);
+      gv = tn_load8(static_cast<const bf16_t*>(Gv) + (long)i * ldg, m0 + (tid & 3) * 8, M, i < N);
+      if constexpr (GT == 3) {
+#pragma unroll
+        for (int e = 0; e < 4; ++e) gv[e] = f16x2_to_bf16x2(gv[e]);
+      }
+    } else if constexpr (GT == 2) {
+      const float* gr = static_cast<const float*>(Gv) + (long)m * ldg + g0;
+      float f[8];
+#pragma unroll
+      for (int e = 0; e < 8; ++e) f[e] = 0.f;
+      if (ok && col + 8 <= N) {
+        const f32x4 a = *reinterpret_cast<const f32x4*>(gr + col), b = *reinterpret_cast<const f32x4*>(gr + col + 4);
+#pragma unroll
+        for (int e = 0; e < 4; ++e) { f[e] = a[e]; f[4 + e] = b[e]; }
+      } else if (ok) {
+#pragma unroll
+        for (int e = 0; e < 8; ++e)
+          if (col + e < N) f[e] = gr[col + e];
+      }
+#pragma unroll
+      for (int e = 0; e < 8; ++e) bsum[e] += f[e];
+#pragma unroll
+      for (int e = 0; e < 4; ++e) gv[e] = pack_bf16x2(f[2 * e], f[2 * e + 1]);
+    } else {
+      gv = tn_load8(static_cast<const bf16_t*>(Gv) + (long)m * ldg + g0, col, N, ok);
+#pragma unroll
+      for (int e = 0; e < 4; ++e) {
+        bsum[2 * e] += from16_lo<GT != 0>(gv[e]);
+        bsum[2 * e + 1] += from16_hi<GT != 0>(gv[e]);
+        if constexpr (GT == 3) gv[e] = f16x2_to_bf16x2(gv[e]);
+      }
+    }
+  };
+  load(0);
+  for (int m0 = 0; m0 < M; m0 += 32) {
+#pragma unroll
+    for (int c = 0; c < 4; ++c) tn_store8(xt, xc0 + c * 8, xrow, xv[c]);
+    if constexpr (GC) *reinterpret_cast<u32x4*>(&gt[(tid >> 2) * kTnXS + (tid & 3) * 8]) = gv;
+    else tn_store8(gt, gc0, xrow, gv);
+    __syncthreads();
+    if (m0 + 32 < M) load(m0 + 32);
+    tn_mma<GF16>(xt, gt, NB, acc, wave, r16, kq);
+    __syncthreads();
+  }
+#pragma unroll
+  for (int a = 0; a < 4; ++a) {
+#pragma unroll
+    for (int b = 0; b < 4; ++b) {
+      const int h = h0 + wave * 64 + b * 16 + r16;
+#pragma unroll
+      for (int e = 0; e < 4; ++e) {
+        const int i = i0 + a * 16 + 4 * kq + e;
+        if (a < NB && i < N && h < H) {
+          const long o = coff + (long)i * ldc + h;
+          if (p.out_kind == TCAVT_F32) static_cast<float*>(p.C)[o] = acc[a][b][e];
+          else static_cast<bf16_t*>(p.C)[o] = p.out_kind == TCAVT_F16 ? f32_to_f16(acc[a][b][e]) : f32_to_bf16(acc[a][b][e]);
+        }
+      }
+    }
+  }
+  if (want_b) {
+    float* red = reinterpret_cast<float*>(xt);
+#pragma unroll
+    for (int e = 0; e < 8; ++e) red[xrow * 64 + gc0 + e] = bsum[e];
+    __syncthreads();
+    if (tid < 64 && i0 + tid < N) {
+      float s = 0.f;
+      for (int r = 0; r < 32; ++r) s += red[r * 64 + tid];
+      gb[i0 + tid] = gb_acc ? gb[i0 + tid] + s : s;
     }
   }
 }
@@ -2124,6 +2271,56 @@
   return TCAVT_OK;
 }
 
+namespace {
+int launch_tn(const TnP& p, int g_dtype, int x_dtype, bool gc, int batch, tcavt_stream_t stream) {
+  const dim3 grid((p.H + 255) / 256, (p.N + 63) / 64, batch), block(256);
+  TCAVT_CHECK_ARG(grid.y <= 65535 && batch >= 1 && batch <= 65535, "gemm_tn / gemm_nn: too many row tiles or batches");
+  const bool xf16 = x_dtype == TCAVT_F16;
+  void (*kfn)(TnP);
+  if (gc) {
+    if (g_dtype == TCAVT_BF16) kfn = xf16 ? gemm_tn_kernel<true, 0, true> : gemm_tn_kernel<false, 0, true>;
+    else kfn = xf16 ? gemm_tn_kernel<true, 1, true> : gemm_tn_kernel<false, 3, true>;
+  } else if (g_dtype == TCAVT_F32) kfn = xf16 ? gemm_tn_kernel<true, 2> : gemm_tn_kernel<false, 2>;
+  else if (g_dtype == TCAVT_BF16) kfn = xf16 ? gemm_tn_kernel<true, 0> : gemm_tn_kernel<false, 0>;
+  else kfn = xf16 ? gemm_tn_kernel<true, 1> : gemm_tn_kernel<false, 3>;
+  hipLaunchKernelGGL(kfn, grid, block, 0, static_cast<hipStream_t>(stream), p);
+  TCAVT_CHECK_LAUNCH("gemm_tn");
+  return TCAVT_OK;
+}
+}
+
+extern "C" int tcavt_gemm_tn(const void* G, int64_t ldg, int g_col0, int g_dtype, const void* X, int64_t ldx, int x_dtype, float* C,
+                             int64_t ldc, int N, int H, int M, float* gb, int gb_accumulate, tcavt_stream_t stream) {
+  TCAVT_CHECK_ARG(G && X && C && M > 0 && N > 0 && H > 0 && g_col0 >= 0 && ldc >= H && ldx >= H && ldg >= (int64_t)g_col0 + N,
+                  "gemm_tn: null pointer or bad shape (ldc, ldx >= H; ldg >= g_col0 + N)");
+  TCAVT_CHECK_ARG((g_dtype == TCAVT_F32 || is16(g_dtype)) && is16(x_dtype), "gemm_tn: G is fp32, bf16 or fp16, X bf16 or fp16");
+  const int gal = g_dtype == TCAVT_F32 ? 4 : 8;
+  TCAVT_CHECK_ARG(aligned16(G) && aligned16(X) && ldg % gal == 0 && g_col0 % gal == 0 && ldx % 8 == 0,
+                  "gemm_tn: G, X 16-byte aligned, ldg / g_col0 / ldx multiples of 16 bytes");
+  TnP p = {};
+  p.G = G; p.X = static_cast<const bf16_t*>(X); p.C = C; p.gb = gb; p.ldg = ldg; p.ldx = ldx; p.ldc = ldc; p.g0 = g_col0; p.N = N; p.M = M;
+  p.H = H; p.gb_acc = gb_accumulate; p.out_kind = TCAVT_F32; p.batch_inner = 1;
+  return launch_tn(p, g_dtype, x_dtype, false, 1, stream);
+}
+
+extern "C" int tcavt_gemm_nn(const tcavt_gemm_nn_args* a, tcavt_stream_t stream) {
+  TCAVT_CHECK_ARG(a && a->A && a->X && a->C && a->M > 0 && a->N > 0 && a->K > 0 && a->lda >= a->K && a->ldx >= a->N && a->ldc >= a->N,
+                  "gemm_nn: null pointer or bad shape (lda >= K; ldx, ldc >= N)");
+  TCAVT_CHECK_ARG(is16(a->a_dtype) && is16(a->x_dtype) && (a->out_dtype == TCAVT_F32 || is16(a->out_dtype)),
+                  "gemm_nn: A, X bf16 or fp16; C fp32, bf16 or fp16");
+  TCAVT_CHECK_ARG(aligned16(a->A) && aligned16(a->X) && a->lda % 8 == 0 && a->ldx % 8 == 0, "gemm_nn: A, X 16-byte aligned, lda / ldx %% 8 == 0");
+  const int batch = a->batch > 1 ? a->batch : 1;
+  if (batch > 1)
+    TCAVT_CHECK_ARG(a->batch_inner >= 1 && batch % a->batch_inner == 0 && a->sAo % 8 == 0 && a->sAi % 8 == 0 && a->sXo % 8 == 0 &&
+                        a->sXi % 8 == 0,
+                    "gemm_nn: batch must be a multiple of batch_inner, the A / X batch strides multiples of 8 elements");
+  TnP p = {};
+  p.G = a->A; p.X = static_cast<const bf16_t*>(a->X); p.C = a->C; p.gb = nullptr; p.ldg = a->lda; p.ldx = a->ldx; p.ldc = a->ldc;
+  p.N = a->M; p.M = a->K; p.H = a->N; p.out_kind = a->out_dtype; p.batch_inner = batch > 1 ? a->batch_inner : 1;
+  p.sGo = a->sAo; p.sGi = a->sAi; p.sXo = a->sXo; p.sXi = a->sXi; p.sCo = a->sCo; p.sCi = a->sCi;
+  return launch_tn(p, a->a_dtype, a->x_dtype, true, batch, stream);
+}
+
 extern "C" int tcavt_lora_wgrad_a(const void* x16, const float* part, int npart, float eps, const float* gamma, const void* g_t,
                                   float* dA, int64_t ldc, int M, int H, float dropout_p, uint64_t dropout_seed, uint32_t site_q,
                                   uint32_t site_v, int dtype16, tcavt_stream_t stream) {
diff --git a/traffic-context-augmented-vehicle-trajectory-prediction-framework-using-multimodal-llm_amd/csrc/small.hip b/traffic-context-augmented-vehicle-trajectory-prediction-framework-using-multimodal-llm_amd/csrc/small.hip
--- a/traffic-context-augmented-vehicle-trajectory-prediction-framework-using-multimodal-llm_amd/csrc/small.hip
+++ b/traffic-context-augmented-vehicle-trajectory-prediction-framework-using-multimodal-llm_amd/csrc/small.hip
@@ -17,13 +17,15 @@
   }
 }
 
+template <bool ROWSUM>
 __global__ __launch_bounds__(256) void gemm_f32_kernel(const float* __restrict__ A, long rsA, long csA,
                                                        const float* __restrict__ W, long rsW, long csW,
                                                        const float* __restrict__ bias,
                                                        const float* __restrict__ res, long ldr,
                                                        float* __restrict__ C, long ldc, int M, int N,
                                                        int K, int flags, int k_chunk, DropoutP drop,
-                                                       float* __restrict__ part) {
+                                                       float* __restrict__ part, float* __restrict__ rowsum,
+                                                       int rowsum_acc, float* __restrict__ rs_part) {
   const int kb = blockIdx.z * k_chunk, ke = min(K, kb + k_chunk);
   __shared__ float As[64][17];
   __shared__ float Ws[64][17];
@@ -41,11 +43,13 @@
   gemm_f32_fetch(A, rsA, csA, m0, M, kb, ke, tid, akf, va, ra, ka);
   gemm_f32_fetch(W, rsW, csW, n0, N, kb, ke, tid, wkf, vw, rw, kw);
   const int lr = lane & 15, lk = lane >> 4;
+  float rsum[4] = {0.f, 0.f, 0.f, 0.f};
   for (int k0 = kb; k0 < ke; k0 += 16) {
 #pragma unroll
     for (int e = 0; e < 4; ++e) {
       As[ra[e]][ka[e]] = va[e];
       Ws[rw[e]][kw[e]] = vw[e];
+      if constexpr (ROWSUM) rsum[e] += va[e];
     }
     __syncthreads();
     if (k0 + 16 < ke) {
@@ -65,6 +69,24 @@
         for (int j = 0; j < 2; ++j) acc[i][j] = __builtin_amdgcn_mfma_f32_16x16x4f32(af[i], wf[j], acc[i][j], 0, 0, 0);
     }
     __syncthreads();
+  }
+  if constexpr (ROWSUM) {
+    if (blockIdx.x == 0) {
+      const int nslot = akf ? 16 : 4;
+      if (akf) {
+#pragma unroll
+        for (int e = 0; e < 4; ++e) As[ra[e]][tid & 15] = rsum[e];
+      } else {
+        As[ra[0]][tid >> 6] = ((rsum[0] + rsum[1]) + rsum[2]) + rsum[3];
+      }
+      __syncthreads();
+      if (tid < 64 && m0 + tid < M) {
+        float t = 0.f;
+        for (int i = 0; i < nslot; ++i) t += As[tid][i];
+        if (gridDim.z > 1) rs_part[(long)blockIdx.z * M + m0 + tid] = t;
+        else rowsum[m0 + tid] = rowsum_acc ? rowsum[m0 + tid] + t : t;
+      }
+    }
   }
 #pragma unroll
   for (int i = 0; i < 2; ++i)
@@ -259,8 +281,15 @@
 __global__ __launch_bounds__(256) void splitk_reduce_f32_kernel(const float* __restrict__ part, int S,
                                                                 const float* __restrict__ bias,
                                                                 const float* __restrict__ res, long ldr, float* C,
-                                                                long ldc, int M, int N, int flags) {
+                                                                long ldc, int M, int N, int flags,
+                                                                const float* __restrict__ rs_part, float* __restrict__ rowsum,
+                                                                int rowsum_acc) {
   const long i = (long)blockIdx.x * 256 + threadIdx.x;
+  if (rowsum && i < M) {
+    float t = rs_part[i];
+    for (int s = 1; s < S; ++s) t += rs_part[(long)s * M + i];
+    rowsum[i] = rowsum_acc ? rowsum[i] + t : t;
+  }
   if (i >= (long)M * N) return;
   const int m = (int)(i / N), n = (int)(i % N);
   float v = part[i];
@@ -273,14 +302,15 @@
 
 static int launch_gemm_f32(int max_splits, const float* A, long rsA, long csA, const float* W, long rsW, long csW, const float* bias,
                            const float* residual, long ldr, float* C, long ldc, int M, int N, int K, int flags,
-                           DropoutP drop, float* ws, int64_t ws_elems, hipStream_t stream, const char* what) {
+                           DropoutP drop, float* ws, int64_t ws_elems, hipStream_t stream, const char* what,
+                           float* rowsum = nullptr, int rowsum_acc = 0) {
   const int tiles = ((N + 63) / 64) * ((M + 63) / 64);
   int splits = 1;
   if (tiles < 128 && K >= 512 && !(flags & TCAVT_EPI_RELU) && drop.p == 0.f) {
     int cap = 0;
     if (ws)
-      cap = (int)std::min<int64_t>(max_splits, ws_elems / ((int64_t)M * N));
-    else if (!(flags & TCAVT_EPI_ACCUM) && residual != C && ldc == N)
+      cap = (int)std::min<int64_t>(max_splits, ws_elems / ((int64_t)M * N + (rowsum ? M : 0)));
+    else if (!(flags & TCAVT_EPI_ACCUM) && residual != C && ldc == N && !rowsum)
       cap = std::min(max_splits, 2);
     splits = std::min(K / 256, cap);
     while (splits > 1 && tiles * splits > 512) splits >>= 1;
@@ -300,11 +330,16 @@
     }
   }
   dim3 grid((N + 63) / 64, (M + 63) / 64, splits), block(256);
-  hipLaunchKernelGGL(gemm_f32_kernel, grid, block, 0, stream, A, rsA, csA, W, rsW, csW, bias, residual, ldr, C, ldc, M,
-                     N, K, flags, k_chunk, drop, splits > 1 && partials ? ws : nullptr);
+  float* rs_part = rowsum && splits > 1 ? ws + (int64_t)splits * M * N : nullptr;
+  if (rowsum)
+    hipLaunchKernelGGL(gemm_f32_kernel<true>, grid, block, 0, stream, A, rsA, csA, W, rsW, csW, bias, residual, ldr, C, ldc, M,
+                       N, K, flags, k_chunk, drop, splits > 1 && partials ? ws : nullptr, rowsum, rowsum_acc, rs_part);
+  else
+    hipLaunchKernelGGL(gemm_f32_kernel<false>, grid, block, 0, stream, A, rsA, csA, W, rsW, csW, bias, residual, ldr, C, ldc, M,
+                       N, K, flags, k_chunk, drop, splits > 1 && partials ? ws : nullptr, nullptr, 0, nullptr);
   if (splits > 1 && partials)
     hipLaunchKernelGGL(splitk_reduce_f32_kernel, dim3((unsigned)(((int64_t)M * N + 255) / 256)), dim3(256), 0, stream, ws,
-                       splits, bias, residual, ldr, C, ldc, M, N, flags);
+                       splits, bias, residual, ldr, C, ldc, M, N, flags, rs_part, rs_part ? rowsum : nullptr, rowsum_acc);
   hipError_t e = hipGetLastError();
   if (e != hipSuccess) {
     set_error("%s: launch failed: %s", what, hipGetErrorString(e));
@@ -341,6 +376,16 @@
                          "gemm_f32_strided");
 }
 
+extern "C" int tcavt_gemm_f32_strided_rowsum(const float* A, int64_t rsA, int64_t csA, const float* W, int64_t rsW, int64_t csW,
+                                             float* C, int64_t ldc, int M, int N, int K, int flags, float* rowsum,
+                                             int rowsum_accumulate, float* ws, int64_t ws_elems, tcavt_stream_t stream) {
+  TCAVT_CHECK_ARG(A && W && C && rowsum && M > 0 && N > 0 && K > 0, "gemm_f32_strided_rowsum: null pointer or bad shape");
+  TCAVT_CHECK_ARG(!(flags & ~TCAVT_EPI_ACCUM), "gemm_f32_strided_rowsum: ACCUM is the only flag");
+  return launch_gemm_f32(8, A, (long)rsA, (long)csA, W, (long)rsW, (long)csW, nullptr, nullptr, 0, C, (long)ldc, M, N, K, flags,
+                         make_dropout(0.f, 0, 0), ws, ws_elems, static_cast<hipStream_t>(stream), "gemm_f32_strided_rowsum", rowsum,
+                         rowsum_accumulate);
+}
+
 extern "C" int tcavt_poly_embed(const float* polygon, const float* w_in, const float* b_in,
                                 const float* pos, float* x, int B, int P, int D, tcavt_stream_t stream) {
   TCAVT_CHECK_ARG(polygon && w_in && b_in && pos && x && B > 0 && P > 0 && D > 0, "poly_embed: bad args");
diff --git a/traffic-context-augmented-vehicle-trajectory-prediction-framework-using-multimodal-llm_amd/csrc/tlayers.hip b/traffic-context-augmented-vehicle-trajectory-prediction-framework-using-multimodal-llm_amd/csrc/tlayers.hip
--- a/traffic-context-augmented-vehicle-trajectory-prediction-framework-using-multimodal-llm_amd/csrc/tlayers.hip
+++ b/traffic-context-augmented-vehicle-trajectory-prediction-framework-using-multimodal-llm_amd/csrc/tlayers.hip
@@ -105,8 +105,7 @@
   const float p = f.dropout_p;
   const float scale = (float)(1.0 / sqrt((double)dh));
   auto lin32 = [&](const float* x, const float* W, const float* gy, float* gW, float* gb, float* gx, int Mr, int N, int K) -> int {
-    TCAVT_TRY(tcavt_gemm_f32_strided(gy, 1, N, x, 1, K, nullptr, nullptr, 0, gW, K, N, K, Mr, TCAVT_EPI_ACCUM, a->red_ws, a->red_ws_elems, stream));
-    TCAVT_TRY(tcavt_colsum(gy, N, TCAVT_F32, gb, Mr, N, 1, a->red_ws, a->red_ws_elems, stream));
+    TCAVT_TRY(tcavt_gemm_f32_strided_rowsum(gy, 1, N, x, 1, K, gW, K, N, K, Mr, TCAVT_EPI_ACCUM, gb, 1, a->red_ws, a->red_ws_elems, stream));
     return tcavt_gemm_f32_strided(gy, N, 1, W, 1, K, nullptr, nullptr, 0, gx, K, Mr, K, N, 0, a->red_ws, a->red_ws_elems, stream);
   };
   const float* g_in = a->g_out;
@@ -275,12 +274,32 @@
   return TCAVT_OK;
 }
 
+namespace {
+__global__ __launch_bounds__(256) void f16_to_bf16_rows_kernel(const bf16_t* __restrict__ in, bf16_t* __restrict__ out, int L, int Lp,
+                                                               int H, long total) {
+  const long idx = (long)blockIdx.x * 256 + threadIdx.x;
+  if (idx >= total) return;
+  const int h8 = H >> 3;
+  const long row = idx / h8;
+  const int c = (int)(idx - row * h8) * 8;
+  const long b = row / Lp;
+  const int r = (int)(row - b * Lp);
+  u32x4 v = {0u, 0u, 0u, 0u};
+  if (r < L) {
+    v = *reinterpret_cast<const u32x4*>(in + (b * L + r) * H + c);
+#pragma unroll
+    for (int e = 0; e < 4; ++e) v[e] = pack_bf16x2(from16_lo<true>(v[e]), from16_hi<true>(v[e]));
+  }
+  *reinterpret_cast<u32x4*>(out + row * H + c) = v;
+}
+}
+
 extern "C" int tcavt_cross_attn_backward(const tcavt_cross_attn_bwd_args* a, tcavt_stream_t stream) {
-  TCAVT_CHECK_ARG(a && a->fwd && a->g_att && a->w_in && a->gw_in && a->gb_in && a->g_q && a->fh_tb && a->fh_b && a->ga_t &&
-                      a->g_ctx && a->w_t && a->x_t && a->d_p && a->d_s && a->g_qp,
+  TCAVT_CHECK_ARG(a && a->fwd && a->g_att && a->w_in && a->gw_in && a->gb_in && a->g_q && a->fh_b && a->g_ctx && a->w_t && a->d_p &&
+                      a->d_s && a->g_qp,
                   "cross_attn_backward: null pointer");
   const tcavt_cross_attn_args& f = *a->fwd;
-  const int B = f.B, To = f.To, L = f.L, Lp = f.Lp, H = f.H, nh = f.nhead, dh = H / nh, M = B * To, Mp = (M + 63) / 64 * 64;
+  const int B = f.B, To = f.To, L = f.L, Lp = f.Lp, H = f.H, nh = f.nhead, dh = H / nh, M = B * To;
   TCAVT_CHECK_ARG(f.dtype16 == TCAVT_F16 && (f.dropout_p == 0.f || a->p_undropped), "cross_attn_backward: fp16 forward; train mode needs p_undropped");
   const float scale = (float)(1.0 / sqrt((double)dh));
   const int BF = TCAVT_BF16;
@@ -288,7 +307,6 @@
   char* g_ctx = static_cast<char*>(a->g_ctx);
   char* g_qp = static_cast<char*>(a->g_qp);
   char* g_q = static_cast<char*>(a->g_q);
-  char* ga_t = static_cast<char*>(a->ga_t);
   const char* ctx = static_cast<const char*>(f.ctx);
   const char* q = static_cast<const char*>(f.q);
   auto gemm = [&](const void* A, int64_t lda, const void* W, int64_t ldw, void* C, int64_t ldc, int out_dtype, int Mr, int N, int K) {
@@ -296,16 +314,19 @@
     g.A = A; g.lda = lda; g.W = W; g.ldw = ldw; g.C = C; g.ldc = ldc; g.M = Mr; g.N = N; g.K = K; g.out_dtype = out_dtype; g.in_dtype = BF;
     return tcavt_gemm_bf16(&g, stream);
   };
-  TCAVT_TRY(tcavt_transpose16(f.fh, H, a->fh_tb, (int64_t)B * Lp, L, H, Lp, B, (int64_t)L * H, Lp, 1, stream));
-  TCAVT_TRY(tcavt_transpose16(a->fh_tb, (int64_t)B * Lp, a->fh_b, H, H, B * Lp, H, 1, 0, 0, 0, stream));
-  TCAVT_TRY(tcavt_colsum(a->g_att, H, BF, a->gb_in + 2 * H, M, H, 1, a->red_ws, a->red_ws_elems, stream));
-  TCAVT_TRY(tcavt_transpose16(a->g_att, H, a->ga_t, Mp, M, H, Mp, 1, 0, 0, 0, stream));
+  TCAVT_CHECK_ARG(aligned16(f.fh) && aligned16(a->fh_b), "cross_attn_backward: fh / fh_b must be 16-byte aligned");
+  {
+    const long total = (long)B * Lp * (H / 8);
+    hipLaunchKernelGGL(f16_to_bf16_rows_kernel, dim3((unsigned)((total + 255) / 256)), dim3(256), 0, static_cast<hipStream_t>(stream),
+                       static_cast<const bf16_t*>(f.fh), static_cast<bf16_t*>(a->fh_b), L, Lp, H, total);
+    TCAVT_CHECK_LAUNCH("cross_attn_backward: bf16 image of the hidden states");
+  }
   for (int h = 0; h < nh; ++h) {
     const float* Wv_h = a->w_in + (size_t)(2 * H + h * dh) * H;
     TCAVT_TRY(tcavt_transpose_f32_bf16(Wv_h, H, a->w_t, dh, dh, H, dh, stream));
     TCAVT_TRY(gemm(g_att + (size_t)h * dh * 2, H, a->w_t, dh, g_ctx + (size_t)h * M * H * 2, H, BF, M, H, dh));
-    TCAVT_TRY(tcavt_transpose16(ctx + (size_t)h * M * H * 2, H, a->x_t, Mp, M, H, Mp, 1, 0, 0, 1, stream));
-    TCAVT_TRY(gemm(ga_t + (size_t)h * dh * Mp * 2, Mp, a->x_t, Mp, a->gw_in + (size_t)(2 * H + h * dh) * H, H, TCAVT_F32, dh, H, Mp));
+    TCAVT_TRY(tcavt_gemm_tn(a->g_att, H, h * dh, BF, ctx + (size_t)h * M * H * 2, H, TCAVT_F16, a->gw_in + (size_t)(2 * H + h * dh) * H, H,
+                            dh, H, M, a->gb_in + 2 * H + h * dh, 1, stream));
   }
   {
     tcavt_gemm_args g = {};
@@ -323,20 +344,19 @@
   }
   TCAVT_TRY(tcavt_softmax_bwd_rows(p_used, Lp, a->d_p, Lp, a->d_s, Lp, scale, B * nh * To, L, Lp, stream));
   {
-    tcavt_gemm_args g = {};
-    g.A = a->d_s; g.lda = Lp; g.W = a->fh_tb; g.ldw = (int64_t)B * Lp; g.C = a->g_qp; g.ldc = H; g.M = To; g.N = H; g.K = Lp;
-    g.out_dtype = BF; g.in_dtype = BF; g.tile = 64; g.batch = B * nh; g.batch_inner = nh;
-    g.sAo = (int64_t)nh * To * Lp; g.sAi = (int64_t)To * Lp; g.sWo = Lp; g.sWi = 0;
+    tcavt_gemm_nn_args g = {};
+    g.A = a->d_s; g.lda = Lp; g.X = f.fh; g.ldx = H; g.C = a->g_qp; g.ldc = H; g.M = To; g.N = H; g.K = L;
+    g.a_dtype = BF; g.x_dtype = TCAVT_F16; g.out_dtype = BF; g.batch = B * nh; g.batch_inner = nh;
+    g.sAo = (int64_t)nh * To * Lp; g.sAi = (int64_t)To * Lp; g.sXo = (int64_t)L * H; g.sXi = 0;
     g.sCo = (int64_t)To * H; g.sCi = (int64_t)M * H;
-    TCAVT_TRY(tcavt_gemm_bf16(&g, stream));
+    TCAVT_TRY(tcavt_gemm_nn(&g, stream));
   }
   for (int h = 0; h < nh; ++h) {
     const float* Wk_h = a->w_in + (size_t)(H + h * dh) * H;
     TCAVT_TRY(tcavt_cast_f32_16(Wk_h, a->w_t, (int64_t)dh * H, BF, stream));
     TCAVT_TRY(gemm(g_qp + (size_t)h * M * H * 2, H, a->w_t, H, g_q + (size_t)h * dh * 2, H, BF, M, dh, H));
-    TCAVT_TRY(tcavt_transpose16(q + (size_t)h * dh * 2, H, a->ga_t, Mp, M, dh, Mp, 1, 0, 0, 1, stream));
-    TCAVT_TRY(tcavt_transpose16(g_qp + (size_t)h * M * H * 2, H, a->x_t, Mp, M, H, Mp, 1, 0, 0, 0, stream));
-    TCAVT_TRY(gemm(a->ga_t, Mp, a->x_t, Mp, a->gw_in + (size_t)(H + h * dh) * H, H, TCAVT_F32, dh, H, Mp));
+    TCAVT_TRY(tcavt_gemm_tn(q, H, h * dh, TCAVT_F16, g_qp + (size_t)h * M * H * 2, H, BF, a->gw_in + (size_t)(H + h * dh) * H, H, dh, H, M,
+                            nullptr, 0, stream));
   }
   return TCAVT_OK;
 }
@@ -363,14 +383,13 @@
                       f.poly_dim > 0,
                   "ltsf_backward: bad shape");
   TCAVT_CHECK_ARG(f.dropout_p >= 0.f && f.dropout_p < 1.f, "ltsf_backward: dropout_p must be in [0, 1)");
-  const int B = f.B, C = f.C, T = f.T, To = f.To, H = f.H, Mo = B * To, Mt = B * T, CT = C * To, Mp = (Mo + 63) / 64 * 64;
+  const int B = f.B, C = f.C, T = f.T, To = f.To, H = f.H, Mo = B * To, Mt = B * T, CT = C * To;
   const float p = f.dropout_p;
   const uint64_t seed = f.dropout_seed;
   const uint32_t s0 = f.first_site;
   const int BF = TCAVT_BF16;
   auto lin32 = [&](const float* x, const float* W, const float* gy, float* gW, float* gb, float* gx, int M, int N, int K) -> int {
-    TCAVT_TRY(tcavt_gemm_f32_strided(gy, 1, N, x, 1, K, nullptr, nullptr, 0, gW, K, N, K, M, TCAVT_EPI_ACCUM, a->red_ws, a->red_ws_elems, stream));
-    TCAVT_TRY(tcavt_colsum(gy, N, TCAVT_F32, gb, M, N, 1, a->red_ws, a->red_ws_elems, stream));
+    TCAVT_TRY(tcavt_gemm_f32_strided_rowsum(gy, 1, N, x, 1, K, gW, K, N, K, M, TCAVT_EPI_ACCUM, gb, 1, a->red_ws, a->red_ws_elems, stream));
     if (gx) TCAVT_TRY(tcavt_gemm_f32_strided(gy, N, 1, W, 1, K, nullptr, nullptr, 0, gx, K, M, K, N, 0, a->red_ws, a->red_ws_elems, stream));
     return TCAVT_OK;
   };
@@ -381,13 +400,7 @@
       TCAVT_TRY(tcavt_cast_f32_16(static_cast<const float*>(gy), a->s_gyb, (int64_t)Mo * N, BF, stream));
       gyb = a->s_gyb;
     }
-    TCAVT_TRY(tcavt_transpose16(gyb, N, a->s_gyt, Mp, Mo, N, Mp, 1, 0, 0, 0, stream));
-    TCAVT_TRY(tcavt_transpose16(x16, K, a->s_xt, Mp, Mo, K, Mp, 1, 0, 0, 1, stream));
-    tcavt_gemm_args g = {};
-    g.A = a->s_gyt; g.lda = Mp; g.W = a->s_xt; g.ldw = Mp; g.C = gW; g.ldc = K; g.M = N; g.N = K; g.K = Mp;
-    g.out_dtype = TCAVT_F32; g.in_dtype = BF;
-    TCAVT_TRY(tcavt_gemm_bf16(&g, stream));
-    TCAVT_TRY(tcavt_colsum(gy, N, gy_dtype, gb, Mo, N, 1, a->red_ws, a->red_ws_elems, stream));
+    TCAVT_TRY(tcavt_gemm_tn(gy, N, 0, gy_dtype, x16, K, TCAVT_F16, gW, K, N, K, Mo, gb, 1, stream));
     TCAVT_TRY(tcavt_transpose_f32_bf16(W, K, a->s_wt, N, N, K, N, stream));
     tcavt_gemm_args d = {};
     d.A = gyb; d.lda = N; d.W = a->s_wt; d.ldw = N; d.C = gx; d.ldc = K; d.M = Mo; d.N = K; d.K = N;
@@ -406,7 +419,7 @@
     TCAVT_CHECK_ARG(a->g_out_w && a->g_out_b && a->g_fl3_w && a->g_fl3_b && a->g_fl1_w && a->g_fl1_b && a->g_fl_n_w && a->g_fl_n_b &&
                         a->g_un_w && a->g_un_b && a->g_co_w && a->g_co_b && a->g_dp_w && a->g_dp_b && a->g_lane_w && a->g_lane_b &&
                         a->g_poly && a->g_f2 && a->g_f1 && a->g_fn && a->g_dec_t && a->g_dt2 && a->g_cross && a->g_proj && a->g_d1 &&
-                        a->s_gyb && a->s_gyt && a->s_xt && a->s_wt,
+                        a->s_gyb && a->s_wt,
                     "ltsf_backward: phase 1: null gradient pointer / workspace");
     TCAVT_CHECK_ARG(a->xattn.fwd == &f.xattn, "ltsf_backward: xattn.fwd must point at fwd->xattn");
     TCAVT_TRY(tcavt_out_head_bwd(a->g_out, f.f2, f.out_w, a->g_f2, a->g_out_w, a->g_out_b, B, To, C, f.F, stream));
diff --git a/traffic-context-augmented-vehicle-trajectory-prediction-framework-using-multimodal-llm_amd/ops.py b/traffic-context-augmented-vehicle-trajectory-prediction-framework-using-multimodal-llm_amd/ops.py
--- a/traffic-context-augmented-vehicle-trajectory-prediction-framework-using-multimodal-llm_amd/ops.py
+++ b/traffic-context-augmented-vehicle-trajectory-prediction-framework-using-multimodal-llm_amd/ops.py
@@ -798,6 +798,43 @@
                                float(rs_eps), stream_ptr()), "tcavt_wgrad_tn")
 
 
+def gemm_nn(a, x, out, *, M, N, K, lda, ldx, ldc, batch=1, inner=1, sA=(0, 0), sX=(0, 0), sC=(0, 0)):
+    if a.dtype not in _H16 or x.dtype not in _H16 or out.dtype not in _DT:
+        raise capi.TcavtError("gemm_nn: a, x bf16 / fp16; out fp32 / bf16 / fp16")
+    g = capi.GemmNnArgs()
+    g.A, g.X, g.C, g.lda, g.ldx, g.ldc, g.M, g.N, g.K = ptr(a).value, ptr(x).value, ptr(out).value, lda, ldx, ldc, M, N, K
+    g.a_dtype, g.x_dtype, g.out_dtype, g.batch, g.batch_inner = _DT[a.dtype], _DT[x.dtype], _DT[out.dtype], batch, inner
+    (g.sAo, g.sAi), (g.sXo, g.sXi), (g.sCo, g.sCi) = sA, sX, sC
+    check(lib().tcavt_gemm_nn(ctypes.byref(g), stream_ptr()), "tcavt_gemm_nn")
+
+
+def gemm_f32_wgrad_bias(gy, x, gW, gb, accumulate=True, ws=None):
+    for t, nm in ((gy, "gy"), (x, "x"), (gW, "gW"), (gb, "gb")):
+        _req(t, torch.float32, "gemm_f32_wgrad_bias." + nm)
+    M, N = gy.shape
+    K = x.shape[1]
+    if x.shape[0] != M or tuple(gW.shape) != (N, K) or gy.stride(1) != 1 or x.stride(1) != 1 or not gW.is_contiguous() or gb.numel() < N:
+        raise capi.TcavtError("gemm_f32_wgrad_bias: operand shapes / strides")
+    check(lib().tcavt_gemm_f32_strided_rowsum(ptr(gy), 1, gy.stride(0), ptr(x), 1, x.stride(0), ptr(gW), K, N, K, M,
+                                              capi.EPI_ACCUM if accumulate else 0, ptr(gb), int(bool(accumulate)),
+                                              ptr(ws) if ws is not None else None, ws.numel() if ws is not None else 0, stream_ptr()),
+          "tcavt_gemm_f32_strided_rowsum")
+
+
+def gemm_tn(g, x, out, gb=None, accumulate_gb=False):
+    if g.dtype not in _DT or x.dtype not in _H16 or out.dtype != torch.float32 or g.dim() != 2 or x.dim() != 2 or out.dim() != 2:
+        raise capi.TcavtError("gemm_tn: g fp32 / bf16 / fp16 [M, N], x bf16 / fp16 [M, H], out fp32 [N, H]")
+    M, N = g.shape
+    H = x.shape[1]
+    if x.shape[0] != M or tuple(out.shape) != (N, H) or g.stride(1) != 1 or x.stride(1) != 1 or out.stride(1) != 1:
+        raise capi.TcavtError("gemm_tn: operand shapes / strides")
+    if gb is not None:
+        _req(gb, torch.float32, "gemm_tn.gb")
+        _need(gb, N, "gemm_tn.gb")
+    check(lib().tcavt_gemm_tn(ptr(g), g.stride(0), 0, _DT[g.dtype], ptr(x), x.stride(0), _DT[x.dtype], ptr(out), out.stride(0), N, H, M,
+                              ptr(gb) if gb is not None else None, int(bool(accumulate_gb)), stream_ptr()), "tcavt_gemm_tn")
+
+
 def lora_wgrad_a(x16, part, gamma, g_t, dA, eps, dropout=None, site_v=None):
     _req16(x16, "lora_wgrad_a.x16")
     _req16(g_t, "lora_wgrad_a.g_t", like=x16)
```

Result: slower. 2177 (-1.4%).
